# 10XGenomics/rust-pseudoaligner

Measured on AMD Instinct MI355X. Metric: reads/sec pseudoaligned (whole node) on synthetic 150bp reads, higher is better.
Workload: dtype u64; 1 GPU; config3: ~202k-transcript synthetic GENCODE-scale index (K=24), error-free 150bp reads; read_len=150, k=24, transcripts=201914, kmers=103866252, index_bytes=7185579820

## Files before the change

### __graft_entry__.py

```python
from __future__ import annotations

import importlib
import sys
from pathlib import Path

ROOT = Path(__file__).resolve().parent
for p in (str(ROOT), str(ROOT / "tests")):
    if p not in sys.path:
        sys.path.insert(0, p)


def build() -> None:
    _b = importlib.import_module("rust-pseudoaligner_amd._build")
    _b.build_product()
    _b.build_maxbins_variant()
    _b.build_abi_check()
    import helpers
    helpers.build_all()
    pa = helpers.pa
    assert pa.lib().pa_abi_version() == 1


def smoke() -> None:
    import numpy as np
    import helpers
    pa = helpers.pa
    if pa.lib().pa_device_count() < 1:
        raise RuntimeError("smoke() needs a GPU: %s" % pa.lib().pa_last_error().decode())
    host = pa.build_index(str(helpers.FASTA), 20, 8)
    aligner = pa.Pseudoaligner(host, 0)
    ids, seqs = helpers.read_fastq()
    res, coff, cids = aligner.map_batch(seqs)
    o_res, o_coff, o_ids, _ = helpers.Oracle(host).map_reads(seqs, 2, 4)
    helpers.assert_same_as_oracle(res, coff, cids, o_res, o_coff, o_ids, "smoke small.fq K=20")
    r = aligner.map_read("GGCTGTCAACCAGTCCATAGGCAGGGCCATCAGGCACCAAAGGGATTCTGCCAGCATAGT")
    assert r == ([1, 30], 60), r
    print("smoke ok: %d reads bit-exact vs oracle, %d mapped" % (len(seqs), int((res["mismatches"] >> 31).sum())))


if __name__ == "__main__":
    build()
    if "--smoke" in sys.argv:
        smoke()
```

### rust-pseudoaligner_amd/_build.py

```python
from __future__ import annotations

import os
import shutil
import subprocess
from pathlib import Path

PKG = Path(__file__).resolve().parent
ROOT = PKG.parent
CSRC = PKG / "csrc"

PRODUCT_SO = PKG / "libpseudoaligner_amd.so"

HOST_SOURCES = ["host_index.cpp", "dbg_build.cpp", "device_flatten.cpp", "synth.cpp", "fastq_text.cpp", "fastq_reads.cpp", "pair_reader.cpp", "fastq_cells.cpp", "fastq_pairs.cpp", "record_stream.cpp", "host_batch.cpp", "bgzf.cpp", "bus_host.cpp", "bus_correct_host.cpp", "bus_knee_host.cpp", "genes_host.cpp", "window_feed.cpp", "text_window.cpp"]
HIP_SOURCES = ["kernels.hip", "map_pool.hip", "device_index.hip", "map_batch.hip", "device_plumbing.hip", "collective.hip", "barcode_counts.hip", "index_build.hip", "index_fill.hip", "count_sort.hip", "resolve.hip", "render.hip", "fastq_scan.hip", "compact.hip", "quant.hip", "quant_boot.hip", "pairs.hip", "strands.hip", "inflate.hip", "bus.hip", "pair_scan.hip", "genes.hip", "bus_correct.hip", "bus_knee.hip"]


EXTRA_FLAGS = {"map_pool.hip": ["-mllvm", "-disable-machine-sink"]}


def _stale(target: Path, sources) -> bool:
    if not target.exists():
        return True
    t = target.stat().st_mtime
    return any(Path(s).stat().st_mtime > t for s in sources)


def _run(cmd):
    proc = subprocess.run(cmd, capture_output=True, text=True)
    if proc.returncode != 0:
        raise RuntimeError("build failed: %s\n%s\n%s" % (" ".join(map(str, cmd)), proc.stdout, proc.stderr))
    return proc


def hipcc_path() -> str:
    for cand in (shutil.which("hipcc"), "/opt/rocm/bin/hipcc"):
        if cand and os.path.exists(cand):
            return cand
    raise RuntimeError("hipcc not found: the product library cannot be built")


OBJ_DIR = PKG / "_build"


def _deps_of(src: Path):
    return [src] + list(CSRC.glob("*.hpp")) + list(CSRC.glob("*.inc")) + [ROOT / "include" / "pseudoaligner_amd.h", Path(__file__)]


def build_product(force: bool = False) -> Path:
    from concurrent.futures import ThreadPoolExecutor
    srcs = [CSRC / s for s in HOST_SOURCES + HIP_SOURCES]
    OBJ_DIR.mkdir(exist_ok=True)
    hipcc = hipcc_path()
    flags = ["--offload-arch=gfx950", "-O3", "-std=c++17", "-fPIC", "-pthread", "-Wall", "-Wno-unused-function"]
    jobs = []
    for s in srcs:
        obj = OBJ_DIR / (s.name + ".o")
        if force or _stale(obj, _deps_of(s)):
            jobs.append([hipcc] + flags + EXTRA_FLAGS.get(s.name, []) + ["-x", "hip", "-c", str(s), "-o", str(obj)])
    if jobs:
        with ThreadPoolExecutor(max_workers=min(len(jobs), os.cpu_count() or 1)) as ex:
            list(ex.map(_run, jobs))
    objs = [OBJ_DIR / (s.name + ".o") for s in srcs]
    if jobs or _stale(PRODUCT_SO, objs):
        _run([hipcc, "--offload-arch=gfx950", "-shared", "-fPIC", "-pthread"] + [str(o) for o in objs] + ["-ldl", "-lz", "-o", str(PRODUCT_SO)])
    return PRODUCT_SO


MAXBINS_SO = OBJ_DIR / "libpseudoaligner_amd_maxbins2.so"


def build_maxbins_variant(force: bool = False) -> Path:
    build_product()
    hipcc = hipcc_path()
    src = CSRC / "count_sort.hip"
    obj = OBJ_DIR / "count_sort.maxbins2.o"
    if force or _stale(obj, _deps_of(src)):
        _run([hipcc, "--offload-arch=gfx950", "-O3", "-std=c++17", "-fPIC", "-pthread", "-Wall", "-Wno-unused-function", "-DPA_MAX_BINS=2", "-x", "hip", "-c", str(src), "-o", str(obj)])
    objs = [OBJ_DIR / (s + ".o") for s in HOST_SOURCES + HIP_SOURCES if s != "count_sort.hip"] + [obj]
    if force or _stale(MAXBINS_SO, objs):
        _run([hipcc, "--offload-arch=gfx950", "-shared", "-fPIC", "-pthread"] + [str(o) for o in objs] + ["-ldl", "-lz", "-o", str(MAXBINS_SO)])
    return MAXBINS_SO


ABI_CHECK_SRC = ROOT / "integration" / "c" / "abi_check.c"
ABI_CHECK_BIN = ROOT / "integration" / "c" / "abi_check"


def build_abi_check(force: bool = False) -> Path:
    if force or _stale(ABI_CHECK_BIN, [ABI_CHECK_SRC, ROOT / "include" / "pseudoaligner_amd.h", PRODUCT_SO]):
        _run(["gcc", "-std=c11", "-O1", "-Wall", "-Wextra", "-Werror", "-I", str(ROOT / "include"), str(ABI_CHECK_SRC), "-L", str(PKG),
              "-lpseudoaligner_amd", "-Wl,-rpath," + str(PKG), "-Wl,-rpath,$ORIGIN/../../rust-pseudoaligner_amd", "-o", str(ABI_CHECK_BIN)])
    return ABI_CHECK_BIN


if __name__ == "__main__":
    import sys
    if "--list" in sys.argv:
        for s in HOST_SOURCES + HIP_SOURCES:
            print(" ".join([s] + EXTRA_FLAGS.get(s, [])))
    else:
        print(build_product("--force" in sys.argv))
```

### rust-pseudoaligner_amd/csrc/device_flatten.cpp

```cpp
#include "device_flatten.hpp"

#include <algorithm>
#include <atomic>
#include <thread>

#include "dict_slots.hpp"
#include "lane_steps.hpp"
#include "pa_common.hpp"

#ifndef PA_BRANCH_TAILS
#define PA_BRANCH_TAILS 1
#endif

namespace pa {

DevIndexView FlatDevice::host_view() const {
    DevIndexView v;
    v.table = table.data();
    v.nbuckets = nbuckets;
    v.blobs = blobs.data();
    v.ledge = ledge.data();
    v.seg_g = seg_g.data();
    v.seg_nid = seg_nid.data();
    v.ec = ec.data();
    v.class_ref = class_ref.data();
    v.class_len = class_len.data();
    v.wtable = wtable.data();
    v.wbuckets = wbuckets;
    v.kmask = kmer_mask(k);
    v.kmask_hi = k > 32 ? kmer_mask(k - 32) : 0;
    v.k = k;
    v.num_nodes = num_nodes;
    v.num_classes = num_classes;
    v.num_segs = (uint32_t)seg_g.size();
    v.stream_nt = 0;
    v.bitmap_min = bitmap_min;
    v.bitmap_words = bitmap_words;
    return v;
}

namespace {

template <class F>
void par_ranges(int threads, uint64_t n, F f) {
    if (threads <= 1 || n < 4096) { f(0, n, 0); return; }
    std::vector<std::thread> th;
    for (int t = 0; t < threads; ++t) th.emplace_back([=] { f(n * t / threads, n * (t + 1) / threads, t); });
    for (auto& x : th) x.join();
}

template <class KT> struct Dict;

template <>
struct Dict<u128> {
    static constexpr double LOAD = 1.0 / 3.0;
    static constexpr uint32_t SLOTS = 2;
    uint32_t* words;
    uint64_t nbuckets;
    uint64_t bucket_of(u128 kmer) const { return ((pa_mix128((uint64_t)kmer, (uint64_t)(kmer >> 64)) >> 32) * (uint64_t)(uint32_t)nbuckets) >> 32; }
    void insert_mt(u128 kmer, uint32_t handle, uint32_t off) {
        uint64_t b = bucket_of(kmer);
        for (;;) {
            uint32_t* line = words + b * BUCKET_WORDS;
            for (uint32_t i = 0; i < SLOTS; ++i) {
                uint32_t expect = NO_HANDLE;
                if (__atomic_compare_exchange_n(&line[8 * i + 4], &expect, handle, false, __ATOMIC_RELAXED, __ATOMIC_RELAXED)) {
                    line[8 * i] = (uint32_t)kmer; line[8 * i + 1] = (uint32_t)(kmer >> 32);
                    line[8 * i + 2] = (uint32_t)(kmer >> 64); line[8 * i + 3] = (uint32_t)(kmer >> 96);
                    line[8 * i + 5] = off;
                    return;
                }
            }
            if (++b == nbuckets) b = 0;
        }
    }
    void insert_rest_mt(u128, uint32_t, uint32_t) {}
    bool find(u128 kmer, uint32_t& handle, uint32_t& off, uint32_t* probes_out = nullptr) const {
        uint64_t b = bucket_of(kmer);
        for (uint64_t probes = 0; probes < nbuckets; ++probes) {
            const uint32_t* line = words + b * BUCKET_WORDS;
            bool full = true;
            for (uint32_t i = 0; i < SLOTS; ++i) {
                if (line[8 * i + 4] == NO_HANDLE) { full = false; continue; }
                if (line[8 * i] == (uint32_t)kmer && line[8 * i + 1] == (uint32_t)(kmer >> 32) && line[8 * i + 2] == (uint32_t)(kmer >> 64) &&
                    line[8 * i + 3] == (uint32_t)(kmer >> 96)) {
                    handle = line[8 * i + 4];
                    off = line[8 * i + 5];
                    if (probes_out) *probes_out = (uint32_t)probes;
                    return true;
                }
            }
            if (!full) return false;
            if (++b == nbuckets) b = 0;
        }
        return false;
    }
};

struct HostAtomics {
    static bool cas(uint32_t* p, uint32_t expect, uint32_t v) { return __atomic_compare_exchange_n(p, &expect, v, false, __ATOMIC_RELAXED, __ATOMIC_RELAXED); }
    static void and_(uint32_t* p, uint32_t m) { __atomic_fetch_and(p, m, __ATOMIC_RELAXED); }
};

template <>
struct Dict<uint64_t> {
    static constexpr double LOAD = DICT_LOAD;
    static constexpr uint32_t SLOTS = SLOTS_PER_BUCKET;
    uint32_t* words;
    uint64_t nbuckets;
    void insert_mt(uint64_t kmer, uint32_t handle, uint32_t off) { dict_insert_home<HostAtomics>(words, (uint32_t)nbuckets, kmer, handle, off); }
    void insert_rest_mt(uint64_t kmer, uint32_t handle, uint32_t off) { dict_insert_rest<HostAtomics>(words, (uint32_t)nbuckets, kmer, handle, off); }
    bool find(uint64_t kmer, uint32_t& handle, uint32_t& off, uint32_t* probes_out = nullptr) const {
        uint32_t probes = 0;
        const bool found = dict_find64(words, (uint32_t)nbuckets, kmer, handle, off, probes);
        if (probes_out) *probes_out = probes;
        return found;
    }
};

}

template <class KT>
struct KmerMap {
    std::vector<KT> keys;
    std::vector<uint32_t> vals;
    uint64_t mask;
    explicit KmerMap(uint32_t n) {
        uint64_t cap = 16;
        while (cap < 2ull * n + 2) cap <<= 1;
        keys.assign(cap, 0);
        vals.assign(cap, NO_HANDLE);
        mask = cap - 1;
    }
    void insert(KT km, uint32_t v) {
        for (uint64_t j = KmerOps<KT>::hash(km) & mask;; j = (j + 1) & mask) {
            if (vals[j] == NO_HANDLE) { keys[j] = km; vals[j] = v; return; }
            if (keys[j] == km) return;
        }
    }
    uint32_t find(KT km) const {
        for (uint64_t j = KmerOps<KT>::hash(km) & mask;; j = (j + 1) & mask) {
            if (vals[j] == NO_HANDLE) return NO_HANDLE;
            if (keys[j] == km) return vals[j];
        }
    }
};

template <class KT>
static int flatten_t(const pa_flat_index& f, int threads, FlatDevice& out, bool device_dict) {
    if (threads < 1) threads = 1;
    const uint32_t k = f.k, N = f.num_nodes;
    out = FlatDevice();
    out.k = k;
    out.num_nodes = N;
    out.num_classes = f.num_classes;
    const KT mask = KmerOps<KT>::mask(k);
    const uint32_t topshift = 2 * (k - 1);

    if (f.num_transcripts >= 0xFFFFFFFFu) return fail(PA_ERR_UNSUPPORTED, "too many transcripts");
    std::vector<U4> cwin(f.num_classes, U4{0, 0, 0, 0});
    uint64_t nwin = 0;
    for (uint32_t c = 0; c < f.num_classes; ++c) {
        const uint32_t* ids = f.ec_ids + f.ec_offset[c];
        const uint64_t len = f.ec_offset[c + 1] - f.ec_offset[c];
        if (len == 0) continue;
        U4 w{ids[0], 0, 0, 0};
        uint64_t j = 0;
        for (; j < len && ids[j] - w.x < CLASS_WINDOW; ++j) w.y |= 1u << (ids[j] - w.x);
        if (j < len) {
            w.z = ids[j];
            for (; j < len && ids[j] - w.z < CLASS_WINDOW; ++j) w.w |= 1u << (ids[j] - w.z);
        }
        if (j < len) continue;
        cwin[c] = w;
        ++nwin;
    }
    uint32_t id_span = f.num_transcripts;
    for (uint64_t j = 0; j < f.ec_offset[f.num_classes]; ++j) id_span = std::max(id_span, f.ec_ids[j] + 1u);
    out.bitmap_words = ((id_span + 31) / 32 + 2 + 3) & ~3u;
    out.bitmap_min = 16;
    for (;;) {
        uint64_t n = 0;
        for (uint32_t c = 0; c < f.num_classes; ++c)
            n += cwin[c].y == 0 && f.ec_offset[c + 1] - f.ec_offset[c] >= out.bitmap_min;
        out.num_bitmaps = n;
        if (n * out.bitmap_words * 4ull <= (4ull << 30)) break;
        if (out.bitmap_min >= (1u << 24)) { out.bitmap_min = 0; out.num_bitmaps = 0; break; }
        out.bitmap_min *= 2;
    }
    out.class_ref.resize(f.num_classes);
    out.class_len.resize(f.num_classes);
    for (uint32_t c = 0; c < f.num_classes; ++c) {
        const uint64_t len = f.ec_offset[c + 1] - f.ec_offset[c];
        if (len >= 0xFFFFFFFFull || out.ec.size() / 4 >= 0xFFFFFFFFull) return fail(PA_ERR_UNSUPPORTED, "class id lists too large");
        out.class_ref[c] = (uint32_t)(out.ec.size() / 4);
        out.class_len[c] = (uint32_t)len;
        out.max_class_len = std::max(out.max_class_len, (uint32_t)len);
        out.ec.push_back(c);
        out.ec.insert(out.ec.end(), f.ec_ids + f.ec_offset[c], f.ec_ids + f.ec_offset[c + 1]);
        while (out.ec.size() % 4 || out.ec.size() - 4ull * out.class_ref[c] < 8) out.ec.push_back(0xFFFFFFFFu);
        if (out.bitmap_min && cwin[c].y == 0 && len >= out.bitmap_min) {
            const size_t at = out.ec.size();
            if (at != class_bitmap(out.class_ref[c], (uint32_t)len)) return fail(PA_ERR_INTERNAL, "class record of %llu ids is not %u chunks", (unsigned long long)len, class_record_chunks((uint32_t)len));
            out.ec.resize(at + out.bitmap_words, 0u);
            for (uint64_t j = f.ec_offset[c]; j < f.ec_offset[c + 1]; ++j) {
                out.ec[at + (f.ec_ids[j] >> 5)] |= 1u << (f.ec_ids[j] & 31u);
            }
        }
    }
    out.ec.resize(out.ec.size() + 8, 0xFFFFFFFFu);
    out.wbuckets = (uint32_t)std::max<uint64_t>(1, (uint64_t)((double)nwin / (WT_ENTRIES * 0.5)) + 1);
    out.wtable.assign((size_t)out.wbuckets * 16, 0);
    for (uint64_t l = 0; l < out.wbuckets; ++l) out.wtable[l * 16 + 4] = out.wtable[l * 16 + 9] = out.wtable[l * 16 + 14] = NO_CLASS;
    for (uint32_t c = 0; c < f.num_classes; ++c) {
        const U4 w = cwin[c];
        if (w.y == 0) continue;
        uint64_t line = ((uint64_t)window_hash(w.x, w.y, w.z, w.w) * out.wbuckets) >> 32;
        for (bool done = false; !done;) {
            uint32_t* e = out.wtable.data() + line * 16;
            for (uint32_t t = 0; t < WT_ENTRIES && !done; ++t)
                if (e[5 * t + 4] == NO_CLASS) {
                    e[5 * t] = w.x; e[5 * t + 1] = w.y; e[5 * t + 2] = w.z; e[5 * t + 3] = w.w; e[5 * t + 4] = c;
                    done = true;
                }
            if (++line == out.wbuckets) line = 0;
        }
    }

    std::vector<uint64_t> seq_pad(f.node_seq, f.node_seq + (f.seq_bases + 31) / 32);
    seq_pad.resize(seq_pad.size() + 3, 0);
    const uint64_t* node_seq = seq_pad.data();
    uint64_t nk = 0;
    for (uint32_t i = 0; i < N; ++i) {
        if (f.node_len[i] < k) return fail(PA_ERR_FORMAT, "node %u shorter than k", i);
        if (f.node_len[i] >= (1u << 24)) return fail(PA_ERR_UNSUPPORTED, "node %u longer than 2^24 bases", i);
        if (f.node_colour[i] >= f.num_classes) return fail(PA_ERR_FORMAT, "node %u: colour out of range", i);
        nk += f.node_len[i] - k + 1;
    }
    out.num_kmers = nk;
    std::vector<uint32_t> redge(4ull * N, NO_HANDLE), ledge_n(4ull * N, NO_HANDLE);
    {
        KmerMap<KT> first_of(N), last_of(N);
        if (!f.node_redge || !f.node_ledge)
            for (uint32_t i = 0; i < N; ++i) {
                first_of.insert(KmerOps<KT>::get(node_seq, f.node_start[i], k), i);
                last_of.insert(KmerOps<KT>::get(node_seq, f.node_start[i] + f.node_len[i] - k, k), i);
            }
        std::atomic<uint32_t> dangling{NO_HANDLE};
        par_ranges(threads, N, [&](uint64_t a, uint64_t b, int) {
            for (uint64_t i = a; i < b; ++i) {
                const uint64_t s = f.node_start[i];
                const KT first = KmerOps<KT>::get(node_seq, s, k), last = KmerOps<KT>::get(node_seq, s + f.node_len[i] - k, k);
                for (uint32_t base = 0; base < 4; ++base) {
                    if (f.node_exts[i] & (1u << base)) {
                        const uint32_t t = f.node_redge ? f.node_redge[4 * i + base] : first_of.find((last >> 2) | ((KT)base << topshift));
                        if (t >= N) dangling.store((uint32_t)i);
                        else redge[4 * i + base] = t;
                    }
                    if (f.node_exts[i] & (1u << (4 + base))) {
                        const uint32_t t = f.node_ledge ? f.node_ledge[4 * i + base] : last_of.find(((first << 2) | (KT)base) & mask);
                        if (t >= N) dangling.store((uint32_t)i);
                        else ledge_n[4 * i + base] = t;
                    }
                }
            }
        });
        if (dangling.load() != NO_HANDLE)
// ... 108 lines not shown
                        const uint64_t c = 1 + shared_ids(f.node_colour[cur], f.node_colour[t]);
                        if (c > best) { best = c; bn = t; }
                    }
                }
                if (bn == NO_HANDLE) break;
                const uint64_t sb = (uint64_t)fin.back().e - (k - 1), full = sb + f.node_len[bn];
                if ((uint64_t)fin.back().e + 1 >= limit) break;
                const bool cut = full > limit;
                fin.back().branch = branch;
                if (!fits_after(fin, c0, SegI{bn, (uint32_t)sb, (uint32_t)(cut ? limit : full), cut})) { fin.back().branch = false; break; }
                if (cut) break;
                cur = bn;
            }
            for (const size_t c1 = c0 + (chain_first[c + 1] - chain_first[c]); fin.size() > c1 && !fin.back().link;) {
                const uint32_t re = f.node_exts[fin.back().node] & 15u;
                if (re == 0 || (re & (re - 1)) || out.node_s[redge[4 * fin.back().node + (uint32_t)__builtin_ctz(re)]] == 0) break;
                bool done = false;
                if (fin.back().e >= fin[fin.size() - 2].e + 2) {
                    SegI g = fin.back();
                    g.e -= 1;
                    g.link = true;
                    fin.pop_back();
                    done = fits_after(fin, c0, g);
                    if (!done) { g.e += 1; g.link = false; fin.push_back(g); }
                }
                if (!done) { fin.pop_back(); fin.back().branch = false; }
            }
        }
        fin_first.push_back((uint32_t)fin.size());
        segs.swap(fin);
        chain_first.swap(fin_first);
    }
    const size_t nsegs = segs.size();

    std::vector<uint32_t> chain_handle(nchains);
    out.seg_g.resize(nsegs);
    out.seg_nid.resize(nsegs);
    uint64_t cursor = 0;
    for (uint32_t c = 0; c < nchains; ++c) {
        if (cursor >= NO_HANDLE - 8) return fail(PA_ERR_UNSUPPORTED, "graph exceeds the 512 GiB chain address space");
        chain_handle[c] = (uint32_t)cursor;
        for (uint32_t t = chain_first[c]; t < chain_first[c + 1]; ++t) {
            out.seg_g[t] = ((uint64_t)cursor << CH_STRIDE_LOG2) + segs[t].s;
            out.seg_nid[t] = segs[t].node;
        }
        cursor += (segs[chain_first[c + 1] - 1].e + CH_STRIDE - 1) >> CH_STRIDE_LOG2;
    }
    for (uint32_t i = 0; i < N; ++i) out.handle[i] = chain_handle[out.handle[i]];
    const uint64_t nblocks = cursor;
    out.blobs.assign(nblocks * CH_BLOCK + 64, 0);

    std::atomic<uint32_t> bad_edge{NO_HANDLE}, bad_slots{NO_HANDLE};
    par_ranges(threads, nchains, [&](uint64_t ca, uint64_t cb, int) {
        std::vector<uint64_t> cs;
        for (uint64_t c = ca; c < cb; ++c) {
            const uint32_t t0 = chain_first[c], t1 = chain_first[c + 1], clen = segs[t1 - 1].e;
            cs.assign((clen + 31) / 32 + 9, 0);
            for (uint32_t t = t0; t < t1; ++t) {
                const SegI& g = segs[t];
                const uint64_t src = f.node_start[g.node];
                for (uint32_t o = t == t0 ? 0 : k - 1; g.s + o < g.e; ++o) set_base(cs.data(), g.s + o, get_base(node_seq, src + o));
            }
            const uint32_t nblk = (clen + CH_STRIDE - 1) >> CH_STRIDE_LOG2;
            uint32_t tlo = t0;
            for (uint32_t j = 0; j < nblk; ++j) {
                const uint32_t base = j << CH_STRIDE_LOG2;
                uint8_t* blk = out.blobs.data() + ((uint64_t)chain_handle[c] + j) * CH_BLOCK;
                uint32_t* sl = reinterpret_cast<uint32_t*>(blk);
                uint64_t* sq = reinterpret_cast<uint64_t*>(blk + CH_SEQ_BYTES);
                while (tlo < t1 && segs[tlo].e <= base) ++tlo;
                uint32_t slot = 0, recmask = 0;
                for (uint32_t t = tlo; t < t1 && segs[t].s < base + CH_WINDOW; ++t) {
                    const SegI& g = segs[t];
                    const U4 cw = cwin[f.node_colour[g.node]];
                    const bool wide = is_wide(g.node), last = t + 1 == t1, reach = g.e - base < CH_WINDOW,
                               edges = ((last && !g.link && has_redge(g.node)) || g.branch) && reach, link = last && g.link && reach;
                    if (slot + 1 + (wide ? 1 : 0) + (edges || link ? 1 : 0) > CH_SLOTS) { bad_slots.store(g.node); break; }
                    recmask |= 1u << slot;
                    uint32_t* r = sl + 4 * slot++;
                    r[0] = std::min<uint32_t>(g.e - base, SEG_E_FAR) | (wide ? SEG_WIDE : 0u) | (last ? SEG_LAST : 0u) | (edges ? SEG_EDGES : 0u) | (link ? SEG_LINK : 0u);
                    r[1] = f.node_colour[g.node]; r[2] = cw.x; r[3] = cw.y;
                    if (wide) {
                        uint32_t* x = sl + 4 * slot++;
                        x[0] = cw.z; x[1] = cw.w; x[2] = out.class_ref[f.node_colour[g.node]]; x[3] = out.class_len[f.node_colour[g.node]];
                    }
                    if (edges) {
                        uint32_t* x = sl + 4 * slot++;
                        for (uint32_t b = 0; b < 4; ++b) {
                            const uint32_t tn = redge[4 * g.node + b];
                            if (tn != NO_HANDLE && out.node_s[tn] != 0) bad_edge.store(g.node);
                            x[b] = tn == NO_HANDLE ? NO_HANDLE : out.handle[tn];
                        }
                    }
                    if (link) {
                        uint32_t* x = sl + 4 * slot++;
                        const uint32_t xt = out.node_s[g.node] + (g.e - g.s), adv = (xt - 1) >> CH_STRIDE_LOG2;
                        x[0] = out.handle[g.node] + adv;
                        x[1] = xt - (adv << CH_STRIDE_LOG2);
                        x[2] = x[3] = 0;
                    }
                }
                sl[0] |= (std::min(j, CH_BACK_MAX) << SEG_BACK_SHIFT) | (recmask << SEG_RECMASK_SHIFT);
                for (uint32_t w = 0; w < CH_WINDOW / 32; ++w) sq[w] = window32(cs.data(), base + 32ull * w);
            }
        }
    });
    if (bad_slots.load() != NO_HANDLE) return fail(PA_ERR_INTERNAL, "node %u: a chain block needs more than its four slots", bad_slots.load());
    par_ranges(threads, nblocks, [&](uint64_t ba, uint64_t bb, int) {
        for (uint64_t b = ba; b < bb; ++b) {
            uint32_t* sl = reinterpret_cast<uint32_t*>(out.blobs.data() + b * CH_BLOCK);
            const uint32_t recmask = sl[0] >> SEG_RECMASK_SHIFT;
            for (uint32_t t = 0; t < CH_SLOTS; ++t) {
                if (!((recmask >> t) & 1u) || !(sl[4 * t] & SEG_LINK)) continue;
                uint32_t* x = sl + 4 * (t + 1 + ((sl[4 * t] & SEG_WIDE) ? 1u : 0u));
                x[2] = of_cur(block_slot_of(out.blobs.data() + (uint64_t)x[0] * CH_BLOCK, x[1] - 1), true);
            }
        }
    });
    if (bad_edge.load() != NO_HANDLE) return fail(PA_ERR_FORMAT, "node %u: a right edge does not lead to the first k-mer of a chain", bad_edge.load());

    out.ledge.assign(8ull * nblocks + 8, NO_HANDLE);
    for (uint32_t c = 0; c < nchains; ++c) {
        const uint32_t a = segs[chain_first[c]].node;
        for (uint32_t b = 0; b < 4; ++b) {
            const uint32_t tn = ledge_n[4 * a + b];
            uint32_t* e = out.ledge.data() + 8ull * chain_handle[c] + 2 * b;
            e[1] = 0;
            if (tn == NO_HANDLE) continue;
            const uint32_t y = out.node_s[tn] + f.node_len[tn] - k;
            const uint32_t jy = y >> CH_STRIDE_LOG2, j = jy > CH_BACK_MAX ? jy - CH_BACK_MAX : 0;
            e[0] = out.handle[tn] + j;
            e[1] = y - (j << CH_STRIDE_LOG2) + 1;
        }
    }

    auto node_kmers = [&](uint32_t i, auto&& fn) {
        const uint64_t s = f.node_start[i];
        const uint32_t n = f.node_len[i] - k + 1;
        KT km = KmerOps<KT>::get(node_seq, s, k);
        for (uint32_t o = 0; o < n; ++o) {
            if (o) km = (km >> 2) | ((KT)get_base(node_seq, s + o + k - 1) << topshift);
            const uint32_t c = out.node_s[i] + o, blk = out.handle[i] + (c >> CH_STRIDE_LOG2);
            fn(km, blk, dict_entry_off(c, o == 0, block_slot_of(out.blobs.data() + (uint64_t)blk * CH_BLOCK, (c & (CH_STRIDE - 1)) + k - 1)));
        }
    };
    Dict<KT> dict{nullptr, 0};
    if (device_dict) {
        out.node_kcum.resize((size_t)N + 1);
        out.node_kcum[0] = 0;
        for (uint32_t i = 0; i < N; ++i) out.node_kcum[i + 1] = out.node_kcum[i] + (f.node_len[i] - k + 1);
    }
    double load0 = Dict<KT>::LOAD;
    if (const char* v = knob_str("PA_DICT_LOAD")) { const double x = atof(v); if (x > 0.01 && x <= 0.95) load0 = x; }
    for (double load = load0; !device_dict; load *= 0.75) {
        out.nbuckets = std::max<uint64_t>(1, (uint64_t)((double)nk / (Dict<KT>::SLOTS * load)) + 1);
        if (out.nbuckets >= 0xFFFFFFFFull) return fail(PA_ERR_UNSUPPORTED, "dictionary exceeds 2^32 buckets");
        out.table.assign(out.nbuckets * BUCKET_WORDS, 0xFFFFFFFFu);
        dict = Dict<KT>{out.table.data(), out.nbuckets};
        par_ranges(threads, N, [&](uint64_t a, uint64_t b, int) {
            for (uint64_t i = a; i < b; ++i) node_kmers((uint32_t)i, [&](KT km, uint32_t h, uint32_t o) { dict.insert_mt(km, h, o); });
        });
        par_ranges(threads, N, [&](uint64_t a, uint64_t b, int) {
            for (uint64_t i = a; i < b; ++i) node_kmers((uint32_t)i, [&](KT km, uint32_t h, uint32_t o) { dict.insert_rest_mt(km, h, o); });
        });
        std::atomic<uint32_t> bad{NO_HANDLE}, far{0};
        par_ranges(threads, N, [&](uint64_t a, uint64_t b, int) {
            for (uint64_t i = a; i < b; ++i)
                node_kmers((uint32_t)i, [&](KT km, uint32_t h, uint32_t o) {
                    uint32_t fh, fo, probes = 0;
                    if (!dict.find(km, fh, fo, &probes) || fh != h || fo != o) bad.store((uint32_t)i);
                    if (probes > DICT_MAX_PROBES) far.store(1);
                });
        });
        if (bad.load() != NO_HANDLE) return fail(PA_ERR_FORMAT, "a k-mer of node %u occurs twice in the graph", bad.load());
        if (!far.load()) break;
    }
    return PA_OK;
}

int flatten_for_device(const pa_flat_index& f, int threads, FlatDevice& out, bool device_dict) {
    if (f.k < PA_MIN_K || f.k > PA_MAX_K) return fail(PA_ERR_UNSUPPORTED, "k=%u outside [%u,%u]", f.k, PA_MIN_K, PA_MAX_K);
    return f.k <= 32 ? flatten_t<uint64_t>(f, threads, out, device_dict) : flatten_t<u128>(f, threads, out, device_dict);
}

}
```

### rust-pseudoaligner_amd/csrc/device_flatten.hpp

```cpp
#pragma once
#include <vector>

#include "device_layout.hpp"
#ifdef __HIPCC__
#include "hip_buffer.hpp"
#endif

namespace pa {

struct FlatDevice {
    std::vector<uint32_t> table;
    uint64_t nbuckets = 0;
    std::vector<uint8_t> blobs;
    std::vector<uint32_t> handle;
    std::vector<uint32_t> node_s;
    std::vector<uint32_t> ledge;
    std::vector<uint64_t> seg_g;
    std::vector<uint32_t> seg_nid;
    uint32_t num_chains = 0;
    std::vector<uint32_t> ec;
    std::vector<uint32_t> class_ref, class_len;
    std::vector<uint32_t> wtable;
    uint32_t wbuckets = 0;
    uint64_t num_kmers = 0;
    uint32_t k = 0, num_nodes = 0, num_classes = 0, max_class_len = 0;
    uint32_t bitmap_min = 0, bitmap_words = 0;
    uint64_t num_bitmaps = 0;
    std::vector<uint64_t> node_kcum;
    DevIndexView host_view() const;
};

int flatten_for_device(const pa_flat_index& f, int threads, FlatDevice& out, bool device_dict = false);

#ifdef __HIPCC__
int device_fill_index(const FlatDevice& fd, const uint8_t* d_blobs, DeviceBuffer<uint32_t>& table, uint64_t* nbuckets);
#endif

}
```

### rust-pseudoaligner_amd/csrc/device_index.hip

```cpp
#include <hip/hip_runtime.h>

#include <algorithm>
#include <cstdlib>
#include <cstring>
#include <thread>

#include "device_flatten.hpp"
#include "device_index.hpp"
#include "lane_steps.hpp"

using namespace pa;

namespace {

uint64_t list_hash_host(const uint32_t* v, uint32_t n) {
    uint64_t h = 0x243f6a8885a308d3ull ^ n;
    for (uint32_t i = 0; i < n; ++i) h = mix64(h ^ v[i]) + 0x9e3779b97f4a7c15ull;
    return h;
}

}

namespace pa {

void LaunchCtx::release() {
    if (side) (void)hipStreamSynchronize(side);
    ctl.release();
    for (DeviceBuffer<uint32_t>* b : {&spill, &trace, &novel, &keys, &keys_sorted, &keys_ctl, &defer}) b->release();
    for (hipEvent_t e : {ev0, ev1, ev2, ev3, fork, join})
        if (e) (void)hipEventDestroy(e);
    ev0 = ev1 = ev2 = ev3 = fork = join = nullptr;
    if (side) (void)hipStreamDestroy(side);
    side = nullptr;
    timed = false;
}

void* Parked::take(std::mutex& mu) {
    std::lock_guard<std::mutex> g(mu);
    if (held.empty()) return nullptr;
    void* obj = held.back().first;
    held.pop_back();
    return obj;
}
void Parked::put(std::mutex& mu, void* obj, void (*free_fn)(void*)) {
    {
        std::lock_guard<std::mutex> g(mu);
        if (held.size() < cap) {
            held.emplace_back(obj, free_fn);
            return;
        }
    }
    free_fn(obj);
}

void index_host_classes(const pa_index* idx, const uint32_t** ec, const uint32_t** class_ref, int* device) {
    *ec = idx->h_ec.data();
    *class_ref = idx->h_class_ref.data();
    *device = idx->device;
}
void index_pair_view(pa_index* idx, PairIndexView* out) {
    std::lock_guard<std::mutex> g(idx->mu);
    *out = PairIndexView{idx->dv, idx->d_class_table.get(), idx->class_table_size, idx->ovf, idx->device, idx->num_cus};
}
void index_host_class_text(pa_index* idx, const uint64_t** off, const char** text) {
    std::call_once(idx->class_text_once, [idx] {
        const uint32_t nc = idx->stats.num_classes;
        const uint32_t* ec = idx->h_ec.data();
        const uint32_t* cref = idx->h_class_ref.data();
        auto digits = [](uint32_t v) { uint32_t d = 1; while (v >= 10) { v /= 10; ++d; } return d; };
        std::vector<uint64_t>& off_v = idx->h_class_text_off;
        off_v.assign((size_t)nc + 1, 0);
        const int T = std::max(1, std::min(16, usable_threads()));
        const uint32_t* clen = idx->h_class_len.data();
        auto ids_of = [&](uint32_t c, const uint32_t*& ids, uint32_t& n) {
            ids = ec + 4ull * cref[c] + 1;
            n = clen[c];
        };
        {
            std::vector<std::thread> th;
            for (int t = 0; t < T; ++t)
                th.emplace_back([&, t] {
                    for (uint64_t c = (uint64_t)nc * t / T; c < (uint64_t)nc * (t + 1) / T; ++c) {
                        const uint32_t* ids; uint32_t n;
                        ids_of((uint32_t)c, ids, n);
                        uint64_t len = n ? 2ull * (n - 1) : 0;
                        for (uint32_t j = 0; j < n; ++j) len += digits(ids[j]);
                        off_v[c + 1] = len;
                    }
                });
            for (auto& x : th) x.join();
        }
        for (uint32_t c = 0; c < nc; ++c) off_v[c + 1] += off_v[c];
        idx->h_class_text.resize(off_v[nc] + 16);
        {
            std::vector<std::thread> th;
            for (int t = 0; t < T; ++t)
                th.emplace_back([&, t] {
                    for (uint64_t c = (uint64_t)nc * t / T; c < (uint64_t)nc * (t + 1) / T; ++c) {
                        const uint32_t* ids; uint32_t n;
                        ids_of((uint32_t)c, ids, n);
                        char* o = idx->h_class_text.data() + off_v[c];
                        for (uint32_t j = 0; j < n; ++j) {
                            if (j) { *o++ = ','; *o++ = ' '; }
                            char b[10]; int k = 10; uint32_t v = ids[j];
                            do { b[--k] = (char)('0' + v % 10); v /= 10; } while (v);
                            memcpy(o, b + k, (size_t)(10 - k)); o += 10 - k;
                        }
                    }
                });
            for (auto& x : th) x.join();
        }
    });
    *off = idx->h_class_text_off.data();
    *text = idx->h_class_text.data();
}
int index_device_class_text(pa_index* idx, const uint64_t** d_off, const uint8_t** d_text) {
    const uint64_t* off = nullptr;
    const char* txt = nullptr;
    index_host_class_text(idx, &off, &txt);
    std::lock_guard<std::mutex> g(idx->mu);
    if (!idx->d_class_text.get()) {
        if (hipSetDevice(idx->device) != hipSuccess) return fail(PA_ERR_HIP, "hipSetDevice failed");
        int e = upload(idx->d_class_text_off, off, idx->h_class_text_off.size());
        if (e == PA_OK) e = upload(idx->d_class_text, reinterpret_cast<const uint8_t*>(txt), idx->h_class_text.size());
        if (e != PA_OK) return e;
    }
    *d_off = idx->d_class_text_off.get();
    *d_text = idx->d_class_text.get();
    return PA_OK;
}
void* index_take_ingest_cache(pa_index* idx) { return idx->ingest_caches.take(idx->mu); }
void index_put_ingest_cache(pa_index* idx, void* cache, void (*free_fn)(void*)) { idx->ingest_caches.put(idx->mu, cache, free_fn); }
void* index_take_host_pipe(pa_index* idx) { return idx->host_pipes.take(idx->mu); }
void index_put_host_pipe(pa_index* idx, void* pipe, void (*free_fn)(void*)) { idx->host_pipes.put(idx->mu, pipe, free_fn); }

}

extern "C" {

void pa_index_destroy(pa_index* idx) {
    if (!idx) return;
    (void)hipSetDevice(idx->device);
    {
        std::vector<std::pair<void*, void (*)(void*)>> parked;
        { std::lock_guard<std::mutex> g(idx->mu); parked.swap(idx->ingest_caches.held); parked.insert(parked.end(), idx->host_pipes.held.begin(), idx->host_pipes.held.end()); idx->host_pipes.held.clear(); }
        for (auto& c : parked) c.second(c.first);
    }
    for (auto& kv : idx->ctxs) kv.second->release();
    delete idx;
}

int pa_index_create(const pa_flat_index* flat, int device, pa_index** out) {
    if (!flat || !out) return fail(PA_ERR_INVALID_ARG, "null argument");
    int rc = use_device(device);
    if (rc != PA_OK) return rc;
    FlatDevice fd;
    int threads = usable_threads();
    if (threads < 1) threads = 1;
    rc = flatten_for_device(*flat, threads, fd, true);
    if (rc != PA_OK) return rc;

    std::vector<uint32_t> ctab((size_t)fd.num_classes * 2 + 16, 0xFFFFFFFFu);
    for (uint32_t c = 0; c < fd.num_classes; ++c) {
        uint64_t j = list_hash_host(fd.ec.data() + 4ull * fd.class_ref[c] + 1, fd.class_len[c]) % ctab.size();
        while (ctab[j] != 0xFFFFFFFFu)
            if (++j == ctab.size()) j = 0;
        ctab[j] = c;
    }

    pa_index* idx = new (std::nothrow) pa_index();
    if (!idx) return fail(PA_ERR_OOM, "out of memory");
    idx->device = device;
    hipDeviceProp_t prop;
    if (hipGetDeviceProperties(&prop, device) == hipSuccess) idx->num_cus = prop.multiProcessorCount;
    if (idx->num_cus <= 0) idx->num_cus = 256;
    rc = upload(idx->d_blobs, fd.blobs);
    if (rc == PA_OK) rc = upload(idx->d_ledge, fd.ledge);
    if (rc == PA_OK) rc = device_fill_index(fd, idx->d_blobs.get(), idx->d_table, &fd.nbuckets);
    if (rc == PA_OK) rc = upload(idx->d_seg_g, fd.seg_g);
    if (rc == PA_OK) rc = upload(idx->d_seg_nid, fd.seg_nid);
    if (rc == PA_OK) rc = upload(idx->d_ec, fd.ec);
    if (rc == PA_OK) rc = upload(idx->d_class_ref, fd.class_ref);
    if (rc == PA_OK) rc = upload(idx->d_class_len, fd.class_len);
    if (rc == PA_OK) rc = upload(idx->d_class_table, ctab);
    if (rc == PA_OK) rc = upload(idx->d_wtable, fd.wtable);
    if (rc != PA_OK) { pa_index_destroy(idx); return rc; }
    idx->class_table_size = ctab.size();
    idx->dv = fd.host_view();
    idx->dv.table = idx->d_table.get();
    idx->dv.blobs = idx->d_blobs.get();
    idx->dv.ledge = idx->d_ledge.get();
    idx->dv.seg_g = idx->d_seg_g.get();
    idx->dv.seg_nid = idx->d_seg_nid.get();
    idx->h_ec = fd.ec;
    idx->h_class_ref = fd.class_ref;
    idx->h_class_len = fd.class_len;
    idx->dv.ec = idx->d_ec.get();
    idx->dv.class_ref = idx->d_class_ref.get();
    idx->dv.class_len = idx->d_class_len.get();
    idx->dv.wtable = idx->d_wtable.get();
    idx->dv.stream_nt = (fd.k <= 32 && fd.nbuckets * BUCKET_WORDS * 4 > (512ull << 20)) ? 1u : 0u;
    pa_index_stats& s = idx->stats;
    s.num_kmers = fd.num_kmers;
    s.table_slots = fd.nbuckets * SLOTS_PER_BUCKET;
    s.bytes_table = fd.nbuckets * BUCKET_WORDS * 4;
    s.bytes_graph = fd.blobs.size() + fd.ledge.size() * 4 + fd.seg_g.size() * 12;
    s.bytes_classes = (fd.ec.size() + fd.class_ref.size() + fd.class_len.size() + ctab.size() + fd.wtable.size()) * 4;
    s.bytes_total = s.bytes_table + s.bytes_graph + s.bytes_classes;
    s.num_nodes = fd.num_nodes;
    s.num_classes = fd.num_classes;
    s.k = fd.k;
    s.max_class_len = fd.max_class_len;
    *out = idx;
    return PA_OK;
}

int pa_index_create_multi(const pa_flat_index* flat, const int* devices, int ndev, pa_index** out) {
    if (!flat || !devices || !out || ndev < 1) return fail(PA_ERR_INVALID_ARG, "null argument or ndev < 1");
    for (int i = 0; i < ndev; ++i) out[i] = nullptr;
    for (int i = 0; i < ndev; ++i) {
        for (int j = 0; j < i; ++j)
            if (devices[j] == devices[i]) {
                for (int t = 0; t < i; ++t) { pa_index_destroy(out[t]); out[t] = nullptr; }
                return fail(PA_ERR_INVALID_ARG, "device %d listed twice", devices[i]);
            }
        const int rc = pa_index_create(flat, devices[i], &out[i]);
        if (rc != PA_OK) {
            const std::string why = last_error_ref();
            for (int t = 0; t <= i; ++t) { pa_index_destroy(out[t]); out[t] = nullptr; }
            return fail(rc, "device %d: %s", devices[i], why.c_str());
        }
    }
    return PA_OK;
}

int pa_index_get_stats(const pa_index* idx, pa_index_stats* stats) {
    if (!idx || !stats) return fail(PA_ERR_INVALID_ARG, "null argument");
    *stats = idx->stats;
    return PA_OK;
}

uint32_t pa_words_per_read(uint32_t max_read_len) { return (max_read_len + 31) / 32 ? (max_read_len + 31) / 32 : 1; }
size_t pa_tiles_words(uint64_t n_reads, uint32_t words_per_read) { return (size_t)((n_reads + 63) / 64) * words_per_read * 64; }

int pa_encode_reads_device(const pa_index* idx, const uint8_t* d_ascii, const uint64_t* d_offsets, uint64_t n_reads,
                           uint32_t words_per_read, uint64_t* d_tiles, uint32_t* d_lens, void* stream) {
    if (!idx || !d_ascii || !d_offsets || !d_tiles || !d_lens || words_per_read == 0) return fail(PA_ERR_INVALID_ARG, "null argument");
    PA_HIP_TRY(hipSetDevice(idx->device));
    const int e = launch_encode(d_ascii, d_offsets, n_reads, words_per_read, d_tiles, d_lens, static_cast<hipStream_t>(stream));
    if (e) return fail(PA_ERR_HIP, "encode launch: %s", hipGetErrorString((hipError_t)e));
    return PA_OK;
}

}

namespace pa {

static int env_int(const char* name, int dflt) { return knob_int(name, dflt); }

uint32_t spill_cap_of(uint32_t wpr) { return 256 * wpr + 24; }

static int pool_geometry(pa_index* idx, uint64_t n_reads, uint32_t wpr, uint32_t* grid, size_t* lds, uint32_t* slots) {
    const size_t cu_lds = 160 * 1024 - 4096;
    int per_cu = env_int("PA_MAP_BLOCKS_PER_CU", 3);
    uint32_t S = 0;
    for (; per_cu >= 1; --per_cu) {
        const size_t per_wave = cu_lds / (size_t)per_cu / (PA_MAP_BLOCK / 64);
        const size_t per_slot = pool_slot_bytes(wpr);
        if (per_wave < pool_fixed_bytes() + 64 * per_slot + 16) continue;
        S = (uint32_t)((per_wave - pool_fixed_bytes() - 16) / per_slot);
        break;
    }
    if (S < 64) return fail(PA_ERR_UNSUPPORTED, "reads of %u words do not fit the LDS of a compute unit", wpr);
    if (S > pool_max_slots()) S = pool_max_slots();
    const int want = env_int("PA_POOL_SLOTS", 0);
    if (want >= 64 && (uint32_t)want <= S) S = (uint32_t)want;
    *slots = S;
    *lds = pool_lds_bytes(wpr, S);
    int occ = 0;
    if (pool_kernel_occupancy(*lds, &occ) == 0 && occ >= 1 && occ < per_cu) per_cu = occ;
    const uint64_t ntiles = (n_reads + 63) / 64;
    const uint64_t waves_wanted = (ntiles + 7) / 8;
    uint64_t blocks = (waves_wanted + PA_MAP_BLOCK / 64 - 1) / (PA_MAP_BLOCK / 64);
    const uint64_t cap = (uint64_t)idx->num_cus * per_cu;
    if (blocks > cap) blocks = cap;
    if (blocks < 1) blocks = 1;
    *grid = (uint32_t)blocks;
    return PA_OK;
}

static int ctx_of(pa_index* idx, hipStream_t stream, std::shared_ptr<LaunchCtx>* out) {
    std::lock_guard<std::mutex> g(idx->mu);
    auto it = idx->ctxs.find(stream);
    if (it == idx->ctxs.end()) {
        std::shared_ptr<LaunchCtx> c(new (std::nothrow) LaunchCtx());
        if (!c) return fail(PA_ERR_OOM, "out of memory");
        const int rc = grow(c->ctl, 2);
        if (rc != PA_OK) return rc;
        it = idx->ctxs.emplace(stream, std::move(c)).first;
    }
    *out = it->second;
    return PA_OK;
}

int StreamCtx::open(pa_index* idx, hipStream_t stream) {
    PA_HIP_TRY(hipSetDevice(idx->device));
    const int rc = ctx_of(idx, stream, &cx);
    if (rc != PA_OK) return rc;
    lock = std::unique_lock<std::mutex>(cx->mu);
    return PA_OK;
}

int map_launch_locked(pa_index* idx, LaunchCtx* cx, hipStream_t stream, const MapLaunch& m) {
    const uint64_t n_reads = m.n_reads;
    const uint32_t wpr = m.wpr;
    MapCtl* const ctl = cx->ctl.get();
    if (n_reads >= 0xFFFFFFFFull) return fail(PA_ERR_UNSUPPORTED, "at most 2^32-2 reads per batch");
    if (wpr == 0 || wpr > (PA_MAX_READ_LEN + 31) / 32) return fail(PA_ERR_UNSUPPORTED, "words_per_read %u outside [1,%u]", wpr, (PA_MAX_READ_LEN + 31) / 32);
    uint32_t grid = 0;
    size_t lds = 0;
    uint32_t slots = 64;
    int rc = pool_geometry(idx, n_reads, wpr, &grid, &lds, &slots);
    if (rc != PA_OK) return rc;
    const uint32_t spill_cap = spill_cap_of(wpr);
    {
        const size_t per_block = (size_t)(PA_MAP_BLOCK / 64) * slots * spill_cap * 4 * (m.nodes ? 2 : 1);
        const size_t budget = (size_t)6 << 30;
        if ((size_t)grid * per_block > budget) grid = (uint32_t)std::max<size_t>(1, budget / per_block);
    }
    const size_t lanes = (size_t)grid * (PA_MAP_BLOCK / 64) * slots;
    rc = grow(cx->spill, lanes * spill_cap);
    if (rc != PA_OK) return rc;
    if (m.nodes) { rc = grow(cx->trace, lanes * spill_cap); if (rc != PA_OK) return rc; }
    PA_HIP_TRY(hipMemsetAsync(ctl, 0, sizeof(MapCtl), stream));
    MapParams p{};
    p.ix = idx->dv;
    p.tiles = m.tiles;
    p.lens = m.lens;
    p.uniform_len = m.uniform_len;
    p.n_reads = n_reads;
    p.wpr = wpr;
    p.allowed = m.allowed;
    p.results = m.results;
    p.arena = m.arena;
    p.arena_cap = m.arena_cap > PA_MAX_ARENA_ENTRIES ? PA_MAX_ARENA_ENTRIES : m.arena_cap;
    p.colour_out = m.colour;
    p.arena_top = &ctl->arena_top;
    p.status = &ctl->status;
    p.tile_ctr = &ctl->tile_ctr;
    p.spill = cx->spill.get();
    p.spill_cap = spill_cap;
    const uint64_t counts_len = (uint64_t)idx->stats.num_classes + 3;
    const uint64_t defer_cap = defer_capacity(n_reads, grid * (PA_MAP_BLOCK / 64));
    if ((rc = grow(cx->defer, defer_cap * 8))) return rc;
    p.defer = cx->defer.get();
    p.defer_top = &ctl->defer_top;
    p.defer_cap = defer_cap;
    p.keys_cap = 0;
    uint64_t keys_cap = 0;
    if (m.counts) {
        keys_cap = key_stream_capacity(n_reads, grid * (PA_MAP_BLOCK / 64));
        size_t sorted_bytes = 0, ctl_bytes = 0;
        count_keys_scratch(counts_len, n_reads, keys_cap, defer_cap, &sorted_bytes, &ctl_bytes);
        if ((rc = grow(cx->keys, keys_cap + defer_cap)) || (rc = grow(cx->keys_sorted, (sorted_bytes + 3) / 4)) || (rc = grow(cx->keys_ctl, (ctl_bytes + 3) / 4))) return rc;
        p.keys = cx->keys.get();
        p.keys_top = &ctl->keys_top;
        p.keys_cap = keys_cap;
        p.counts = reinterpret_cast<unsigned long long*>(m.counts);
    }
    p.class_table = idx->d_class_table.get();
    p.class_table_size = idx->class_table_size;
    p.pool_slots = slots;
    p.dbg = env_int("PA_MAP_STATS", 0) ? ctl->stats : nullptr;
    p.ablate = (uint32_t)env_int("PA_MAP_ABLATE", 0);
    pa_overflow* ovf = nullptr;
    { std::lock_guard<std::mutex> g(idx->mu); ovf = idx->ovf; }
    if (m.counts && ovf) {
        const uint64_t want = n_reads + 64;
        rc = grow(cx->novel, want * 2);
        if (rc != PA_OK) return rc;
        p.novel_list = cx->novel.get();
        p.novel_ctr = &ctl->novel_ctr;
        p.novel_cap = want;
        overflow_launch_params(ovf, p);
    }
    p.trace = m.nodes ? cx->trace.get() : nullptr;
// ... 215 lines not shown
```

### rust-pseudoaligner_amd/csrc/device_layout.hpp

```cpp
#pragma once
#include <cstdint>

#include "../../include/pseudoaligner_amd.h"

#if defined(__HIPCC__)
#include <hip/hip_runtime.h>
#define PA_HD __host__ __device__ __forceinline__
#else
#define PA_HD inline
#endif

namespace pa {

constexpr uint32_t NO_HANDLE = 0xFFFFFFFFu;
constexpr uint32_t CH_BLOCK = 128;
constexpr uint32_t CH_STRIDE_LOG2 = 6;
constexpr uint32_t CH_STRIDE = 1u << CH_STRIDE_LOG2;
constexpr uint32_t CH_WINDOW = 256;
constexpr uint32_t CH_SLOTS = 4;
constexpr uint32_t CH_SEQ_BYTES = 64;
constexpr uint32_t CH_BACK_MAX = 3;
constexpr uint32_t SEG_E_MASK = 0xFFFFu, SEG_E_FAR = 0xFFFFu;
constexpr uint32_t SEG_WIDE = 1u << 16, SEG_LAST = 1u << 17, SEG_EDGES = 1u << 18, SEG_LINK = 1u << 19;
constexpr uint32_t CH_TAIL = 128;
constexpr uint32_t SEG_BACK_SHIFT = 20, SEG_RECMASK_SHIFT = 28;
constexpr uint32_t ENT_P_MASK = 63u, ENT_NODE_START = 64u, ENT_BACK_SHIFT = 7, ENT_CUR_SHIFT = 9;
PA_HD uint32_t block_slot_of(const uint8_t* blk, uint32_t y) {
    const uint32_t* sl = reinterpret_cast<const uint32_t*>(blk);
    const uint32_t recmask = sl[0] >> SEG_RECMASK_SHIFT;
    for (uint32_t t = 0; t < CH_SLOTS; ++t)
        if (((recmask >> t) & 1u) && (sl[4 * t] & SEG_E_MASK) > y) return t;
    return 0;
}
PA_HD uint32_t dict_entry_off(uint32_t c, bool node_start, uint32_t slot) {
    const uint32_t j = c >> CH_STRIDE_LOG2;
    return (c & ENT_P_MASK) | (node_start ? ENT_NODE_START : 0u) | ((j < CH_BACK_MAX ? j : CH_BACK_MAX) << ENT_BACK_SHIFT) | (slot << ENT_CUR_SHIFT);
}
constexpr uint32_t CLASS_WINDOW = 32;
constexpr uint32_t SLOTS_PER_BUCKET = 4;
constexpr uint32_t BUCKET_WORDS = 16;
constexpr uint32_t SLOT_WORDS = 4;
constexpr uint32_t SLOT_OFF_MASK = 0xFFFFFFu;
constexpr uint32_t SLOT_FLAG_SHIFT = 24;
constexpr uint32_t SLOT_FLAG_OVERFLOW = 8u;
constexpr double DICT_LOAD = 0.25;
constexpr uint32_t DICT_MAX_PROBES = 15;

struct alignas(16) U4 {
    uint32_t x, y, z, w;
};
struct alignas(8) Q2 {
    uint64_t a, b;
};

constexpr uint32_t WT_ENTRIES = 3;

struct DevIndexView {
    const uint32_t* table;
    uint64_t nbuckets;
    const uint8_t* blobs;
    const uint32_t* ledge;
    const uint64_t* seg_g;
    const uint32_t* seg_nid;
    const uint32_t* ec;
    const uint32_t* class_ref;
    const uint32_t* class_len;
    const uint32_t* wtable;
    uint32_t wbuckets;
    uint64_t kmask;
    uint64_t kmask_hi;
    uint32_t k;
    uint32_t num_nodes, num_classes;
    uint32_t num_segs;
    uint32_t stream_nt;
    uint32_t bitmap_min;
    uint32_t bitmap_words;
};

PA_HD uint32_t class_record_chunks(uint32_t len) { return len < 4 ? 2u : (len + 4) >> 2; }
PA_HD uint64_t class_bitmap(uint32_t ref, uint32_t len) { return 4ull * ((uint64_t)ref + class_record_chunks(len)); }

}
```

### rust-pseudoaligner_amd/csrc/dict_slots.hpp

```cpp
#pragma once
#include "lane_steps.hpp"

namespace pa {

template <class A>
PA_HD bool slot_claim(uint32_t* slot, uint64_t km, uint32_t handle, uint32_t off) {
    if (!A::cas(slot + 2, NO_HANDLE, handle)) return false;
    slot[0] = (uint32_t)km;
    slot[1] = (uint32_t)(km >> 32);
    A::and_(slot + 3, off | ~SLOT_OFF_MASK);
    return true;
}

template <class A>
PA_HD void dict_insert_home(uint32_t* table, uint32_t nbuckets, uint64_t km, uint32_t handle, uint32_t off) {
    uint32_t home;
    const uint32_t b = pa_bucket_home(km, nbuckets, home);
    slot_claim<A>(table + (uint64_t)b * BUCKET_WORDS + SLOT_WORDS * home, km, handle, off);
}

template <class A>
PA_HD void dict_insert_rest(uint32_t* table, uint32_t nbuckets, uint64_t km, uint32_t handle, uint32_t off) {
    uint32_t home;
    uint32_t b = pa_bucket_home(km, nbuckets, home);
    {
        const uint32_t* hs = table + (uint64_t)b * BUCKET_WORDS + SLOT_WORDS * home;
        if (hs[2] != NO_HANDLE && hs[0] == (uint32_t)km && hs[1] == (uint32_t)(km >> 32)) return;
    }
    for (bool first = true;; first = false) {
        uint32_t* line = table + (uint64_t)b * BUCKET_WORDS;
        uint32_t* hs = line + SLOT_WORDS * home;
        if (!first && slot_claim<A>(hs, km, handle, off)) return;
        for (uint32_t i = 0; i < 3; ++i)
            if (slot_claim<A>(line + SLOT_WORDS * ((home + 1 + i) & 3u), km, handle, off)) {
                A::and_(hs + 3, ~(1u << (SLOT_FLAG_SHIFT + i)));
                return;
            }
        A::and_(hs + 3, ~(SLOT_FLAG_OVERFLOW << SLOT_FLAG_SHIFT));
        if (++b == nbuckets) b = 0;
    }
}

PA_HD bool dict_find64(const uint32_t* table, uint32_t nbuckets, uint64_t km, uint32_t& handle, uint32_t& off, uint32_t& probes) {
    uint32_t home;
    uint32_t b = pa_bucket_home(km, nbuckets, home);
    const uint32_t klo = (uint32_t)km, khi = (uint32_t)(km >> 32);
    for (probes = 0; probes < nbuckets; ++probes) {
        const uint32_t* line = table + (uint64_t)b * BUCKET_WORDS;
        const U4 v = *reinterpret_cast<const U4*>(line + SLOT_WORDS * home);
        if (slot_holds(v, klo, khi)) { handle = v.z; off = v.w & SLOT_OFF_MASK; return true; }
        const uint32_t fl = slot_flags(v);
        for (uint32_t c = fl & 7u; c; c &= c - 1) {
            const U4 v2 = *reinterpret_cast<const U4*>(line + SLOT_WORDS * ((home + 1 + pa_ctz32(c)) & 3u));
            if (slot_holds(v2, klo, khi)) { handle = v2.z; off = v2.w & SLOT_OFF_MASK; return true; }
        }
        if (!(fl & SLOT_FLAG_OVERFLOW)) return false;
        if (++b == nbuckets) b = 0;
    }
    return false;
}

}
```

### rust-pseudoaligner_amd/csrc/index_fill.hip

```cpp
#include <hip/hip_runtime.h>
#include <cstdlib>

#include <algorithm>

#include "device_flatten.hpp"
#include "dict_slots.hpp"
#include "hip_buffer.hpp"
#include "lane_steps.hpp"
#include "pa_common.hpp"

namespace pa {
namespace {

__device__ __forceinline__ uint64_t win32(const uint64_t* w, uint32_t pos) {
    const uint32_t i = pos >> 5, s = (pos & 31) * 2;
    return s ? (w[i] >> s) | (w[i + 1] << (64 - s)) : w[i];
}

template <class KT> struct FillOps;
template <> struct FillOps<uint64_t> {
    static constexpr uint32_t SLOTS = SLOTS_PER_BUCKET;
    static constexpr double LOAD = DICT_LOAD;
    __host__ __device__ static uint64_t mask(uint32_t k) { return k >= 32 ? ~0ull : ((1ull << (2 * k)) - 1); }
    __device__ static uint64_t get(const uint64_t* seq, uint32_t o, uint32_t k) { return win32(seq, o) & mask(k); }
};
struct DeviceAtomics {
    __device__ static bool cas(uint32_t* p, uint32_t expect, uint32_t v) { return atomicCAS(p, expect, v) == expect; }
    __device__ static void and_(uint32_t* p, uint32_t m) { atomicAnd(p, m); }
};
template <> struct FillOps<u128> {
    static constexpr uint32_t SLOTS = 2;
    static constexpr double LOAD = 1.0 / 3.0;
    __host__ __device__ static u128 mask(uint32_t k) { return k >= 64 ? ~(u128)0 : (((u128)1 << (2 * k)) - 1); }
    __device__ static u128 get(const uint64_t* seq, uint32_t o, uint32_t k) {
        return ((u128)(win32(seq, o + 32) & FillOps<uint64_t>::mask(k - 32)) << 64) | win32(seq, o);
    }
    __device__ static uint32_t bucket(u128 km, uint32_t nbuckets) { return __umulhi((uint32_t)(pa_mix128((uint64_t)km, (uint64_t)(km >> 64)) >> 32), nbuckets); }
    __device__ static bool try_insert(uint32_t* line, u128 km, uint32_t handle, uint32_t off) {
        for (uint32_t i = 0; i < 2; ++i)
            if (atomicCAS(line + 8 * i + 4, NO_HANDLE, handle) == NO_HANDLE) {
                line[8 * i] = (uint32_t)km; line[8 * i + 1] = (uint32_t)(km >> 32);
                line[8 * i + 2] = (uint32_t)(km >> 64); line[8 * i + 3] = (uint32_t)(km >> 96);
                line[8 * i + 5] = off;
                return true;
            }
        return false;
    }
    __device__ static int look(const uint32_t* line, u128 km, uint32_t& handle, uint32_t& off) {
        bool full = true;
        for (uint32_t i = 0; i < 2; ++i) {
            if (line[8 * i + 4] == NO_HANDLE) { full = false; continue; }
            if (line[8 * i] == (uint32_t)km && line[8 * i + 1] == (uint32_t)(km >> 32) && line[8 * i + 2] == (uint32_t)(km >> 64) &&
                line[8 * i + 3] == (uint32_t)(km >> 96)) {
                handle = line[8 * i + 4];
                off = line[8 * i + 5];
                return 1;
            }
        }
        return full ? 2 : 0;
    }
};

template <class KT>
__device__ __forceinline__ bool dict_find(const uint32_t* table, uint32_t nbuckets, KT km, uint32_t& handle, uint32_t& off, uint32_t& probes);
template <>
__device__ __forceinline__ bool dict_find<uint64_t>(const uint32_t* table, uint32_t nbuckets, uint64_t km, uint32_t& handle, uint32_t& off, uint32_t& probes) {
    return dict_find64(table, nbuckets, km, handle, off, probes);
}
template <>
__device__ __forceinline__ bool dict_find<u128>(const uint32_t* table, uint32_t nbuckets, u128 km, uint32_t& handle, uint32_t& off, uint32_t& probes) {
    uint32_t b = FillOps<u128>::bucket(km, nbuckets);
    for (probes = 0; probes < nbuckets; ++probes) {
        const int r = FillOps<u128>::look(table + (uint64_t)b * BUCKET_WORDS, km, handle, off);
        if (r != 2) return r == 1;
        if (++b == nbuckets) b = 0;
    }
    return false;
}

struct KmerAt {
    uint32_t node, block, off;
    const uint64_t* seq;
    uint32_t rel;
};

__device__ __forceinline__ uint32_t node_of_kmer(const uint64_t* kcum, uint32_t num_nodes, uint64_t g) {
    uint32_t lo = 0, hi = num_nodes - 1;
    while (lo < hi) {
        const uint32_t mid = lo + (hi - lo + 1) / 2;
        if (kcum[mid] <= g) lo = mid; else hi = mid - 1;
    }
    return lo;
}

__device__ __forceinline__ KmerAt kmer_at(const uint8_t* blobs, const uint32_t* handle, const uint32_t* node_s, const uint64_t* kcum, uint32_t num_nodes, uint64_t g, uint32_t k) {
    KmerAt a;
    a.node = node_of_kmer(kcum, num_nodes, g);
    const uint32_t o = (uint32_t)(g - kcum[a.node]), c = node_s[a.node] + o;
    a.block = handle[a.node] + (c >> CH_STRIDE_LOG2);
    a.off = dict_entry_off(c, o == 0, block_slot_of(blobs + (uint64_t)a.block * CH_BLOCK, (c & (CH_STRIDE - 1)) + k - 1));
    a.seq = reinterpret_cast<const uint64_t*>(blobs + (uint64_t)a.block * CH_BLOCK + CH_SEQ_BYTES);
    a.rel = c & (CH_STRIDE - 1);
    return a;
}

template <class KT>
__global__ __launch_bounds__(256) void pa_fill_insert_kernel(const uint8_t* __restrict__ blobs, const uint32_t* __restrict__ handle, const uint32_t* __restrict__ node_s,
                                                             const uint64_t* __restrict__ kcum, uint32_t num_nodes, uint64_t nk, uint32_t k, uint32_t* table,
                                                             uint32_t nbuckets, int pass) {
    const uint64_t g = (uint64_t)blockIdx.x * blockDim.x + threadIdx.x;
    if (g >= nk) return;
    const KmerAt a = kmer_at(blobs, handle, node_s, kcum, num_nodes, g, k);
    const KT km = FillOps<KT>::get(a.seq, a.rel, k);
    if constexpr (sizeof(KT) == 8) {
        if (pass == 0) dict_insert_home<DeviceAtomics>(table, nbuckets, km, a.block, a.off);
        else dict_insert_rest<DeviceAtomics>(table, nbuckets, km, a.block, a.off);
    } else {
        if (pass != 0) return;
        uint32_t b = FillOps<KT>::bucket(km, nbuckets);
        for (;;) {
            if (FillOps<KT>::try_insert(table + (uint64_t)b * BUCKET_WORDS, km, a.block, a.off)) return;
            if (++b == nbuckets) b = 0;
        }
    }
}

template <class KT>
__global__ __launch_bounds__(256) void pa_fill_verify_kernel(const uint8_t* __restrict__ blobs, const uint32_t* __restrict__ handle, const uint32_t* __restrict__ node_s,
                                                             const uint64_t* __restrict__ kcum, uint32_t num_nodes, uint64_t nk, uint32_t k,
                                                             const uint32_t* __restrict__ table, uint32_t nbuckets, uint32_t* __restrict__ flags) {
    const uint64_t g = (uint64_t)blockIdx.x * blockDim.x + threadIdx.x;
    if (g >= nk) return;
    const KmerAt a = kmer_at(blobs, handle, node_s, kcum, num_nodes, g, k);
    const KT km = FillOps<KT>::get(a.seq, a.rel, k);
    uint32_t fh = 0, fo = 0, probes = 0;
    if (!dict_find<KT>(table, nbuckets, km, fh, fo, probes) || fh != a.block || fo != a.off) atomicMin(flags, a.node);
    if (probes > DICT_MAX_PROBES) flags[1] = 1;
}

template <class KT>
int fill_t(const FlatDevice& fd, const uint8_t* d_blobs, DeviceBuffer<uint32_t>& table_out, uint64_t* nbuckets_out) {
    const uint32_t N = fd.num_nodes, k = fd.k;
    const uint64_t nk = fd.num_kmers;
    DeviceBuffer<uint32_t> table, d_handle, d_node_s, d_flags;
    DeviceBuffer<uint64_t> d_kcum;
    int e = d_handle.alloc(N ? N : 1);
    if (e == PA_OK) e = d_node_s.alloc(N ? N : 1);
    if (e == PA_OK) e = d_kcum.alloc((size_t)N + 1);
    if (e == PA_OK) e = d_flags.alloc(4);
    if (e != PA_OK) return e;
    if (N) PA_HIP_TRY(hipMemcpy(d_handle.get(), fd.handle.data(), (size_t)N * 4, hipMemcpyHostToDevice));
    if (N) PA_HIP_TRY(hipMemcpy(d_node_s.get(), fd.node_s.data(), (size_t)N * 4, hipMemcpyHostToDevice));
    PA_HIP_TRY(hipMemcpy(d_kcum.get(), fd.node_kcum.data(), ((size_t)N + 1) * 8, hipMemcpyHostToDevice));
    uint64_t nbuckets = 0;
    double load0 = FillOps<KT>::LOAD;
    {
        size_t free_b = 0, total_b = 0;
        const double dense = sizeof(KT) == 8 ? 0.5 : FillOps<KT>::LOAD;
        if (load0 < dense && hipMemGetInfo(&free_b, &total_b) == hipSuccess && (double)nk / (FillOps<KT>::SLOTS * load0) * BUCKET_WORDS * 4 > (double)free_b / 4) load0 = dense;
    }
    if (const char* v = knob_str("PA_DICT_LOAD")) { const double x = atof(v); if (x > 0.01 && x <= 0.95) load0 = x; }
    for (double load = load0;; load *= 0.75) {
        nbuckets = std::max<uint64_t>(1, (uint64_t)((double)nk / (FillOps<KT>::SLOTS * load)) + 1);
        if (nbuckets >= 0xFFFFFFFFull) return fail(PA_ERR_UNSUPPORTED, "dictionary exceeds 2^32 buckets");
        if ((e = table.alloc(nbuckets * BUCKET_WORDS)) != PA_OK) return e;
        PA_HIP_TRY(hipMemsetAsync(table.get(), 0xFF, nbuckets * BUCKET_WORDS * 4, nullptr));
        const uint32_t init[4] = {NO_HANDLE, 0u, NO_HANDLE, NO_HANDLE};
        PA_HIP_TRY(hipMemcpy(d_flags.get(), init, 16, hipMemcpyHostToDevice));
        if (nk) {
            const dim3 grid((uint32_t)((nk + 255) / 256));
            for (int pass = 0; pass < (sizeof(KT) == 8 ? 2 : 1); ++pass) {
                hipLaunchKernelGGL(pa_fill_insert_kernel<KT>, grid, dim3(256), 0, nullptr, d_blobs, d_handle.get(), d_node_s.get(), d_kcum.get(), N, nk, k,
                                   table.get(), (uint32_t)nbuckets, pass);
                PA_HIP_TRY(hipGetLastError());
            }
            hipLaunchKernelGGL(pa_fill_verify_kernel<KT>, grid, dim3(256), 0, nullptr, d_blobs, d_handle.get(), d_node_s.get(), d_kcum.get(), N, nk, k,
                               table.get(), (uint32_t)nbuckets, d_flags.get());
            PA_HIP_TRY(hipGetLastError());
        }
        uint32_t flags[4];
        PA_HIP_TRY(hipMemcpy(flags, d_flags.get(), 16, hipMemcpyDeviceToHost));
        if (flags[0] != NO_HANDLE) return fail(PA_ERR_FORMAT, "a k-mer of node %u occurs twice in the graph", flags[0]);
        if (!flags[1]) break;
    }
    *nbuckets_out = nbuckets;
    table_out = std::move(table);
    return PA_OK;
}

}

int device_fill_index(const FlatDevice& fd, const uint8_t* d_blobs, DeviceBuffer<uint32_t>& table, uint64_t* nbuckets) {
    return fd.k <= 32 ? fill_t<uint64_t>(fd, d_blobs, table, nbuckets) : fill_t<u128>(fd, d_blobs, table, nbuckets);
}

}
```

### rust-pseudoaligner_amd/csrc/lane_steps_body.hpp

```cpp
#if PA_LS_COMMON
enum : uint32_t { ST_EMPTY = 0, ST_SEEK = 1, ST_FWD = 2, ST_LEFT = 3, ST_ISECT = 4, ST_NONE = 5,
                  ST_F_LIGHT = 6, ST_F_SCAN = 7, ST_F_COOP = 8, ST_F_BITS = 9, ST_F_MASK = 10, ST_COUNT = 11 };
enum : uint32_t { F_FRESH = 1u, F_FIRST_SEEK = 2u, F_LEFT_SEED = 4u, F_SPILL_OVERFLOW = 8u, F_CAREFUL = 16u, F_LISTS = 32u,
                  F_SMALL_BASE = 64u,
                  F_SPEC = 128u };
constexpr uint32_t NO_CLASS = 0xFFFFFFFFu;
constexpr uint32_t LDS_CLASSES = 4;
#endif

#if PA_LS_LANE
#if !PA_LANE_WIDE
struct Lane {
    uint32_t rid;
    uint32_t lk;
    uint32_t cm;
    uint32_t h;
    uint32_t of;
    uint32_t rr;
    uint32_t rm;
    uint32_t ph;
    uint32_t nc;
};
constexpr uint32_t LANE_MAX_READ_LEN = 16383u;
PA_HD uint32_t l_L(const Lane& s) { return s.lk & 0x3FFFu; }
// ... 364 lines not shown
        c.wcand[0] = ec_len;
        if (ec_len <= 8) l_or_flags(s, F_SMALL_BASE);
    }
    *reinterpret_cast<U4*>(c.win) = r;
    if (n < LDS_CLASSES) {
        c.refs[n] = ec_ref;
        c.lens[n] = ec_len;
        c.cids[n] = hd.cid;
    } else {
        const uint32_t o = 4 * (n - LDS_CLASSES);
        if (o + 3 >= c.spill_cap || n >= NC_COL_MASK) { l_or_flags(s, F_SPILL_OVERFLOW); return false; }
        c.spill[o] = ec_ref;
        c.spill[o + 1] = ec_len;
        c.spill[o + 2] = hd.cid;
    }
    s.nc += 1;
    return false;
}

PA_HD void lane_start(Lane& s, uint32_t rid, uint32_t L, uint32_t k) {
    s.rid = rid;
    l_zero(s);
    l_set_lk(s, L, 0, L < k ? ST_NONE : ST_SEEK);
    s.of = F_FIRST_SEEK << 24;
}
PA_HD void restart_lists(Lane& s, uint32_t k) {
    lane_start(s, s.rid, l_L(s), k);
    l_or_flags(s, F_LISTS);
}
PA_HD uint32_t window_todo(const Lane& s) {
    const uint32_t n = l_ncol(s);
    return (n >> 1) == 0 ? 0u : (n & 1u) ? 1u : 2u;
}
#endif
#if PA_LS_COMMON
PA_HD void list_window_mask(const DevIndexView& ix, uint32_t ref, uint32_t len, uint32_t b1, uint32_t b2, uint32_t& m1, uint32_t& m2) {
    const uint32_t* ids = ix.ec + 4ull * ref + 1;
    m1 = m2 = 0;
    for (uint32_t j = 0; j < len; ++j) {
        const uint32_t d1 = ids[j] - b1, d2 = ids[j] - b2;
        if (d1 < CLASS_WINDOW) m1 |= 1u << d1;
        if (d2 < CLASS_WINDOW) m2 |= 1u << d2;
    }
#if !defined(__HIP_DEVICE_COMPILE__)
    if (ix.bitmap_min && len >= ix.bitmap_min) {
        const uint32_t* bits = ix.ec + class_bitmap(ref, len);
        const uint32_t x1 = window_bits(bits, b1), x2 = window_bits(bits, b2);
        if (x1 != m1 || x2 != m2) { m1 = m2 = 0xDEADBEEFu; }
    }
#endif
}
#endif
#if PA_LS_LANE
PA_HD void mask_pending(Lane& s, const DevIndexView& ix, ColRef c) {
    U4 w = *reinterpret_cast<const U4*>(c.win);
    const uint32_t np = l_npend(s);
    uint32_t a1 = w.y, a2 = w.w;
    for (uint32_t i = 0; i < np; ++i) {
        uint32_t m1, m2;
        list_window_mask(ix, c.pend[2 * i], c.pend[2 * i + 1], w.x, w.z, m1, m2);
        a1 &= m1;
        a2 &= m2;
    }
    if (a1 != w.y || a2 != w.w) c.wcand[0] = NO_CLASS;
    w.y = a1;
    w.w = a2;
    *reinterpret_cast<U4*>(c.win) = w;
    s.nc = (s.nc & ~NC_COL_MASK) | 1u;
}
#endif

#if PA_LS_COMMON
struct SeekProbe {
    U4 v;
    uint32_t klo, khi;
    uint32_t pending;
};
struct SeekProbe2 {
    U4 k0, v0, k1, v1;
    uint32_t w0, w1, w2, w3;
};
constexpr uint32_t SK_NAMED = 7u, SK_FULL = 8u, SK_MASK = 15u;
PA_HD uint32_t pa_bucket_home(uint64_t kmer, uint32_t nbuckets, uint32_t& home) {
    uint32_t x = (uint32_t)kmer * 0x9E3779B1u + (uint32_t)(kmer >> 32) * 0x85EBCA77u;
    x ^= x >> 15;
    x *= 0x2C1B3C6Du;
    x ^= x >> 13;
    home = x & 3u;
#if defined(__HIP_DEVICE_COMPILE__)
    return __umulhi(x, nbuckets);
#else
    return (uint32_t)(((uint64_t)x * nbuckets) >> 32);
#endif
}
#endif
#if PA_LS_LANE
PA_HD bool seek_two(const Lane& s, uint32_t K) { return (l_flags(s) & F_SPEC) && l_probe(s) == 0 && l_kp(s) + PA_SEEK_STRIDE <= l_L(s) - K; }
PA_HD uint32_t l_pending(const Lane& s) { return s.rm & SK_MASK; }
PA_HD void seek_issue(const Lane& s, const DevIndexView& ix, ReadRef rd, SeekProbe& q, uint32_t ahead = 0, bool live = true) {
    const uint32_t at = live ? l_kp(s) + ahead : l_kp(s);
    const uint64_t kmer = read_window_in(rd, at) & ix.kmask;
    uint32_t home;
    uint32_t b = pa_bucket_home(kmer, (uint32_t)ix.nbuckets, home) + (ahead ? 0u : l_probe(s));
    if (b >= (uint32_t)ix.nbuckets) b -= (uint32_t)ix.nbuckets;
    q.pending = ahead ? 0u : l_pending(s);
    const uint32_t named = q.pending & SK_NAMED;
    uint32_t slot = named ? (home + 1u + pa_ctz32(named)) & 3u : home;
    if (!live) { b = 0; slot = 0; }
    q.v = ld_stream(reinterpret_cast<const U4*>(ix.table + (uint64_t)b * BUCKET_WORDS + SLOT_WORDS * slot), (PA_NT & 4) || ix.stream_nt);
    q.klo = (uint32_t)kmer;
    q.khi = (uint32_t)(kmer >> 32);
}
#endif
#if PA_LS_COMMON
PA_HD bool slot_holds(const U4& v, uint32_t klo, uint32_t khi) { return v.z != NO_HANDLE && v.x == klo && v.y == khi; }
PA_HD uint32_t slot_flags(const U4& v) { return (~v.w >> SLOT_FLAG_SHIFT) & 15u; }
#endif
#if PA_LS_LANE
PA_HD void seek_finish(Lane& s, uint32_t K, uint32_t h, uint32_t off, bool full, uint32_t probe);
#endif
#if PA_LS_COMMON
PA_HD void seek_eval(const SeekProbe& q, uint32_t& h, uint32_t& off, bool& full, uint32_t& pending) {
    h = NO_HANDLE;
    off = 0;
    const bool hit = slot_holds(q.v, q.klo, q.khi);
    if (hit) { h = q.v.z; off = q.v.w & SLOT_OFF_MASK; }
    const uint32_t named = q.pending & SK_NAMED;
    const uint32_t next = named ? (named & (named - 1u)) | (q.pending & SK_FULL) : slot_flags(q.v);
    pending = hit ? 0u : (next & SK_NAMED) ? next : 0u;
    full = (next & SK_FULL) != 0;
}
#endif
#if PA_LS_LANE
PA_HD bool seek_settle(Lane& s, uint32_t K, const SeekProbe& q, bool more) {
    uint32_t h, off, pending;
    bool full;
    seek_eval(q, h, off, full, pending);
    if (pending) { s.rm = (s.rm & ~SK_MASK) | pending; return true; }
    const uint32_t probe = l_probe(s);
    if (!more || h != NO_HANDLE || (full && probe < DICT_MAX_PROBES)) {
        seek_finish(s, K, h, off, full, probe);
        return true;
    }
    l_set_kp(s, l_kp(s) + PA_SEEK_STRIDE);
    s.rm &= ~SK_MASK;
    s.nc &= ~(15u << NC_PROBE_SHIFT);
    return false;
}
PA_HD void seek_complete(Lane& s, uint32_t K, const SeekProbe& q) { (void)seek_settle(s, K, q, false); }
PA_HD void seek_complete2(Lane& s, uint32_t K, const SeekProbe& q0, bool two, const SeekProbe& q1) {
    if (seek_settle(s, K, q0, two)) return;
    (void)seek_settle(s, K, q1, false);
}
PA_HD void seek_finish(Lane& s, uint32_t K, uint32_t h, uint32_t off, bool full, uint32_t probe) {
    const uint32_t L = l_L(s), kp = l_kp(s);
    s.nc &= ~(15u << NC_PROBE_SHIFT);
    s.rm &= ~SK_MASK;
    if (h != NO_HANDLE) {
        s.h = h;
        const uint32_t fl = l_flags(s), p = (off & ENT_P_MASK) | of_cur((off >> ENT_CUR_SHIFT) & 3u, true);
        const uint32_t thr = L / 5;
        if ((fl & F_FIRST_SEEK) && kp >= thr) {
            const uint32_t back = (off >> ENT_BACK_SHIFT) & CH_BACK_MAX;
            l_set_left_ra(s, kp);
            s.ph = h - back;
            s.rr = (off & ENT_P_MASK) + CH_STRIDE * back + ((off & ENT_NODE_START) ? 1u : 0u);
            s.of = p | (((fl & ~(F_FIRST_SEEK | F_SPEC)) | F_FRESH | F_LEFT_SEED) << 24);
            l_set_st(s, ST_LEFT);
        } else {
            s.of = p | (((fl & ~(F_FIRST_SEEK | F_SPEC)) | F_FRESH) << 24);
            l_set_st(s, ST_FWD);
        }
        return;
    }
    if (full && probe < DICT_MAX_PROBES) {
        s.nc |= (probe + 1) << NC_PROBE_SHIFT;
        return;
    }
    const uint32_t nkp = kp + PA_SEEK_STRIDE;
    l_set_kp(s, nkp);
    l_or_flags(s, F_SPEC);
    if (nkp > L - K) l_set_st(s, l_ncol(s) ? ST_ISECT : ST_NONE);
}
#endif

#if PA_LS_COMMON
PA_HD uint64_t pa_mix128(uint64_t lo, uint64_t hi) { return pa_mix64(lo ^ (pa_mix64(hi) * 0x9e3779b97f4a7c15ull)); }
#endif

#if PA_LS_LANE
PA_HD void seek_issue_k2(const Lane& s, const DevIndexView& ix, ReadRef rd, SeekProbe2& q) {
    const uint32_t kp = l_kp(s), probe = l_probe(s);
    const uint64_t klo = read_window(rd, kp), khi = read_window(rd, kp + 32) & ix.kmask_hi;
#if defined(__HIP_DEVICE_COMPILE__)
    uint32_t b = __umulhi((uint32_t)(pa_mix128(klo, khi) >> 32), (uint32_t)ix.nbuckets) + probe;
#else
    uint32_t b = (uint32_t)(((pa_mix128(klo, khi) >> 32) * (uint32_t)ix.nbuckets) >> 32) + probe;
#endif
    if (b >= (uint32_t)ix.nbuckets) b -= (uint32_t)ix.nbuckets;
    const U4* line = reinterpret_cast<const U4*>(ix.table + (uint64_t)b * BUCKET_WORDS);
    q.k0 = line[0]; q.v0 = line[1]; q.k1 = line[2]; q.v1 = line[3];
    q.w0 = (uint32_t)klo; q.w1 = (uint32_t)(klo >> 32); q.w2 = (uint32_t)khi; q.w3 = (uint32_t)(khi >> 32);
}
PA_HD void seek_complete_k2(Lane& s, uint32_t K, const SeekProbe2& q) {
    const bool h0 = q.k0.x == q.w0 && q.k0.y == q.w1 && q.k0.z == q.w2 && q.k0.w == q.w3 && q.v0.x != NO_HANDLE,
               h1 = q.k1.x == q.w0 && q.k1.y == q.w1 && q.k1.z == q.w2 && q.k1.w == q.w3 && q.v1.x != NO_HANDLE;
    seek_finish(s, K, h0 ? q.v0.x : h1 ? q.v1.x : NO_HANDLE, h0 ? q.v0.y : q.v1.y, q.v0.x != NO_HANDLE && q.v1.x != NO_HANDLE, l_probe(s));
}
PA_HD void seek_step(Lane& s, const DevIndexView& ix, ReadRef rd) {
    const uint32_t K = ix.k;
    if (K > 32) {
        SeekProbe2 q2;
        seek_issue_k2(s, ix, rd, q2);
        seek_complete_k2(s, K, q2);
        return;
    }
    SeekProbe q, q1;
    const bool two = seek_two(s, K);
    seek_issue(s, ix, rd, q);
    seek_issue(s, ix, rd, q1, PA_SEEK_STRIDE, two);
    seek_complete2(s, K, q, two, q1);
}
#endif

#if PA_LS_COMMON
struct FwdLoad {
    U4 s0, s1, s2, s3;
    Q2 s01, s23, s45;
};
constexpr uint32_t CH_SEQ_LAST = CH_WINDOW / 32 - 1;
PA_HD const Q2* fwd_seq_pair(const uint64_t* sq, uint32_t w) { return reinterpret_cast<const Q2*>(sq + (w == CH_SEQ_LAST ? CH_SEQ_LAST - 1 : w)); }
PA_HD uint64_t fwd_seq_first(const Q2& v, uint32_t w) { return w == CH_SEQ_LAST ? v.b : v.a; }
PA_HD bool fwd_next_block(uint32_t& h, uint32_t& x, uint32_t rest) {
    const uint32_t adv = x + rest <= CH_WINDOW ? 0u : (x - 1) >> CH_STRIDE_LOG2;
    h += adv;
    x -= adv << CH_STRIDE_LOG2;
    return adv == 0;
}
#endif
#if PA_LS_LANE
PA_HD void fwd_issue(const Lane& s, const DevIndexView& ix, FwdLoad& f) {
    const uint32_t K = ix.k, L = l_L(s);
    const bool fresh = l_flags(s) & F_FRESH;
    const uint32_t xs = l_off(s) + (fresh ? K : 0u);
    const uint32_t kp0 = l_kp(s) + (fresh ? K : 0u);
    const uint8_t* blk = chain_block(ix, s.h);
    const U4* sp = reinterpret_cast<const U4*>(blk);
    const uint32_t rot = l_cur(s);
    f.s0 = PA_LD(8, sp + rot); f.s1 = PA_LD(8, sp + ((rot + 1) & 3u)); f.s2 = PA_LD(8, sp + ((rot + 2) & 3u)); f.s3 = PA_LD(8, sp + ((rot + 3) & 3u));
    const uint32_t most = pa_min(L - kp0, 128u), nwords = ((xs & 31) + most + 31) >> 5, w0 = xs >> 5;
    const uint64_t* sq = reinterpret_cast<const uint64_t*>(blk + CH_SEQ_BYTES);
    f.s01 = PA_LD(8, fwd_seq_pair(sq, w0));
    f.s23 = f.s45 = Q2{0ull, 0ull};
    if (nwords > 2) f.s23 = PA_LD(8, fwd_seq_pair(sq, w0 + 2));
    if (nwords > 4) f.s45.a = PA_LD(8, sq + (w0 + 4));
}
#endif

#if PA_LS_COMMON
struct DiffMasks {
    uint64_t m0, m1, m2, m3;
    uint32_t p0, p1, p2, p3;
};
PA_HD uint64_t diff_word(const DiffMasks& d, uint32_t w) { return sel4q(w, d.m0, d.m1, d.m2, d.m3); }
PA_HD uint32_t mism_prefix(const DiffMasks& d, uint32_t z) {
    const uint32_t w = z >> 5, r = z & 31u;
    const uint32_t b03 = sel4(w, 0u, d.p0, d.p1, d.p2), base = (w & 4u) ? d.p3 : b03;
    return base + pa_popc64(diff_word(d, w) & ((1ull << (2 * r)) - 1));
}
#endif

#if PA_LS_LANE
template <bool TRACE = false>
PA_HD void fwd_finish_general(Lane& s, const DevIndexView& ix, ReadRef rd, ColRef cols, uint32_t allowed, const FwdLoad& f) {
    const uint32_t K = ix.k, L = l_L(s);
    const uint32_t fl = l_flags(s);
    const bool fresh = fl & F_FRESH, careful = fl & F_CAREFUL;
    uint32_t x = l_off(s) + (fresh ? K : 0u);
    uint32_t kp = l_kp(s) + (fresh ? K : 0u);
    const uint32_t xs = x, kp0 = kp;
    uint32_t snp = s.rr >> 24, cov = l_cov(s), mism = l_mism(s);
    const uint32_t most = pa_min(L - kp0, 128u), nwords = ((xs & 31) + most + 31) >> 5;
    const uint64_t a[5] = {fwd_seq_first(f.s01, xs >> 5), f.s01.b, nwords > 2 ? fwd_seq_first(f.s23, (xs >> 5) + 2) : 0ull, nwords > 2 ? f.s23.b : 0ull,
                           nwords > 4 ? f.s45.a : 0ull};
    const Slots sl{f.s0, f.s1, f.s2, f.s3};
    const bool known = s.of & OF_CUR_KNOWN;
    const uint32_t rot = l_cur(s);
    uint32_t cur = known ? 0u : seg_find(sl, x - 1);
    Seg g = seg_at(sl, cur);
    if (fresh) {
        cov += K;
        if (push_node<TRACE>(s, cols, ix, g, 64ull * s.h + l_off(s))) {
            restart_lists(s, K);
            return;
        }
        snp = 0;
    }
    uint64_t r[5];
    {
        const uint32_t i0 = (kp0 >> 5) * rd.stride, ilast = (rd.wmax - 1) * rd.stride;
#pragma unroll
        for (uint32_t i = 0; i < 5; ++i) r[i] = rd.p[pa_min(i0 + i * rd.stride, ilast)];
    }
    const uint32_t sh_a = (xs & 31) * 2, sh_r = (kp0 & 31) * 2;
    DiffMasks dm;
    dm.m0 = diff_mask(funnel(r[0], r[1], sh_r) ^ funnel(a[0], a[1], sh_a), 32u);
    dm.m1 = most > 32u ? diff_mask(funnel(r[1], r[2], sh_r) ^ funnel(a[1], a[2], sh_a), 32u) : 0ull;
    dm.m2 = most > 64u ? diff_mask(funnel(r[2], r[3], sh_r) ^ funnel(a[2], a[3], sh_a), 32u) : 0ull;
    dm.m3 = most > 96u ? diff_mask(funnel(r[3], r[4], sh_r) ^ funnel(a[3], a[4], sh_a), 32u) : 0ull;
    dm.p0 = pa_popc64(dm.m0); dm.p1 = dm.p0 + pa_popc64(dm.m1); dm.p2 = dm.p1 + pa_popc64(dm.m2); dm.p3 = dm.p2 + pa_popc64(dm.m3);
    const uint32_t lim = careful ? 32u : 128u;
    uint32_t consumed = 0, st = ST_FWD, h = s.h, nfl = fl & ~F_FRESH;
    uint32_t ncur = 0xFFFFFFFFu;
    bool premature = false, hopped = false;
    for (;;) {
        const uint32_t n = pa_min(pa_min(g.e - x, L - kp), lim - consumed);
        uint32_t matched;
        if (!careful) {
            const uint32_t cnt = mism_prefix(dm, consumed + n) - mism_prefix(dm, consumed);
            if (snp + cnt > allowed) { nfl |= F_CAREFUL; break; }
            snp += cnt;
            mism += cnt;
            matched = n;
        } else {
            matched = compare_chunk(n ? dm.m0 & (~0ull >> (64u - 2u * n)) : 0ull, n, allowed, snp, mism, premature);
        }
        x += matched; kp += matched; cov += matched; consumed += matched;
        if (premature) { nfl &= ~F_CAREFUL; st = kp > L - K ? ST_ISECT : ST_SEEK; break; }
        if (kp >= L) { nfl &= ~F_CAREFUL; st = ST_ISECT; break; }
        if (x < g.e) break;
        if (g.flags & SEG_LINK) {
            const U4 lk = slot_at(sl, cur + 1 + ((g.flags & SEG_WIDE) ? 1u : 0u));
            h = lk.x;
            x = lk.y;
            ncur = lk.z;
            hopped = true;
            break;
        }
        nfl &= ~F_CAREFUL;
        if (g.flags & SEG_LAST) {
            uint32_t nh = NO_HANDLE;
            if (g.flags & SEG_EDGES) {
                const U4 ed = slot_at(sl, cur + 1 + ((g.flags & SEG_WIDE) ? 1u : 0u));
                const uint32_t b = read_base(rd, kp);
                nh = sel4(b, ed.x, ed.y, ed.z, ed.w);
            }
            if (nh != NO_HANDLE) {
                h = nh;
                x = 0;
                kp -= K - 1;
                cov -= K - 1;
                nfl |= F_FRESH;
                ncur = of_cur(0u, true);
                hopped = true;
            } else st = kp > L - K ? ST_ISECT : ST_SEEK;
            break;
        }
        if (consumed >= 128u) break;
        const bool branch = (g.flags & SEG_EDGES) != 0;
        {
            if ((diff_word(dm, consumed >> 5) >> (2 * (consumed & 31u))) & 1ull) {
                uint32_t nh = NO_HANDLE;
                if (branch) {
                    const U4 ed = slot_at(sl, cur + 1 + ((g.flags & SEG_WIDE) ? 1u : 0u));
                    nh = sel4(read_base(rd, kp), ed.x, ed.y, ed.z, ed.w);
                }
                if (nh != NO_HANDLE) {
                    h = nh;
                    x = 0;
                    kp -= K - 1;
                    cov -= K - 1;
                    nfl |= F_FRESH;
                    ncur = of_cur(0u, true);
                    hopped = true;
// ... 552 lines not shown
```

### rust-pseudoaligner_amd/csrc/map_pool.hip

```cpp
#include <hip/hip_runtime.h>

#include "kernels.hpp"
#include "lane_steps.hpp"
#include "kernel_utils.hpp"

#ifndef PA_FILL
#define PA_FILL 1
#endif
#ifndef PA_COOP_MIN
#define PA_COOP_MIN 2u
#endif
#ifndef PA_REFILL_ALIGN
#define PA_REFILL_ALIGN 1u
#endif
#ifndef PA_RARE_MIN
#define PA_RARE_MIN 16u
#endif

#ifdef PA_ISA_MARKS
#define PA_MARK(name) asm volatile("; PA_MARK " name ::: "memory")
#else
#define PA_MARK(name)
#endif

namespace pa {
namespace {

typedef __attribute__((address_space(3))) uint64_t* lds_u64;
typedef __attribute__((address_space(3))) uint32_t* lds_u32;
typedef __attribute__((address_space(3))) uint8_t* lds_u8;
typedef __attribute__((address_space(3))) uint16_t* lds_u16;
typedef __attribute__((address_space(3))) unsigned long long* lds_u64w;
typedef uint32_t u32x4 __attribute__((ext_vector_type(4)));
typedef __attribute__((address_space(3))) u32x4* lds_v4;
typedef __attribute__((address_space(1))) u32x4* glb_v4w;
typedef __attribute__((address_space(1))) const u32x4* glb_v4;
typedef __attribute__((address_space(1))) uint32_t* glb_u32w;
typedef __attribute__((address_space(1))) const uint32_t* glb_u32;
typedef __attribute__((address_space(1))) unsigned long long* glb_u64w;
__device__ __forceinline__ void store_result(glb_v4w dst, u32x4 v) {
    if (PA_NT & 2) __builtin_nontemporal_store(v, dst);
    else *dst = v;
}

typedef __attribute__((address_space(4))) const MapParams* karg_ptr;

__device__ __forceinline__ DevIndexView view_of(karg_ptr p) {
    DevIndexView v;
    v.table = p->ix.table; v.nbuckets = p->ix.nbuckets; v.blobs = p->ix.blobs; v.ledge = p->ix.ledge;
    v.seg_g = p->ix.seg_g; v.seg_nid = p->ix.seg_nid; v.ec = p->ix.ec; v.class_ref = p->ix.class_ref; v.class_len = p->ix.class_len;
    v.wtable = p->ix.wtable; v.wbuckets = p->ix.wbuckets; v.kmask = p->ix.kmask; v.kmask_hi = p->ix.kmask_hi; v.k = p->ix.k; v.num_nodes = p->ix.num_nodes; v.num_classes = p->ix.num_classes; v.num_segs = p->ix.num_segs; v.stream_nt = p->ix.stream_nt; v.bitmap_min = p->ix.bitmap_min; v.bitmap_words = p->ix.bitmap_words;
    return v;
}

static_assert(ST_NSTAT == ST_COUNT + 4, "kernels.hpp");
constexpr uint32_t ST_DUAL = ST_COUNT;
constexpr uint32_t POOL_FIXED = 960;
constexpr uint32_t POOL_MAX_SLOTS = 128;
constexpr uint32_t LIST_ROW_HDR = 12;

__device__ __forceinline__ uint32_t rank_in(uint64_t m) { return __builtin_amdgcn_mbcnt_hi((uint32_t)(m >> 32), __builtin_amdgcn_mbcnt_lo((uint32_t)m, 0u)); }

__device__ __forceinline__ uint64_t shfl64(uint64_t v, uint32_t src) {
    return ((uint64_t)(uint32_t)__shfl((int)(v >> 32), (int)src, 64) << 32) | (uint32_t)__shfl((int)v, (int)src, 64);
}

__device__ __forceinline__ uint64_t arena_alloc(uint32_t cnt_alloc, uint32_t lane, karg_ptr p, lds_u64w chunk) {
    const uint32_t incl = wave_incl_scan(cnt_alloc);
    const uint32_t total = (uint32_t)__builtin_amdgcn_readlane((int)incl, 63);
    asm volatile("" ::: "memory");
    unsigned long long chunk_cur = chunk[0];
    if (total > 0) {
        if (chunk_cur + total > chunk[1]) {
            const unsigned long long want = total > PA_ARENA_CHUNK ? total : PA_ARENA_CHUNK;
            unsigned long long base = 0;
            if (lane == 0) base = atomicAdd(p->arena_top, want);
            base = ((unsigned long long)(uint32_t)__builtin_amdgcn_readfirstlane((int)(base >> 32)) << 32) | (uint32_t)__builtin_amdgcn_readfirstlane((int)base);
            chunk_cur = base;
            if (lane == 0) chunk[1] = base + want;
        }
        if (lane == 0) chunk[0] = chunk_cur + total;
    }
    asm volatile("" ::: "memory");
    return chunk_cur + (incl - cnt_alloc);
}

constexpr uint32_t NO_KEY = 0xFFFFFFFFu;
__device__ __forceinline__ void append_keys(uint32_t key, uint32_t lane, karg_ptr p, lds_u32 kchunk) {
    const uint64_t m = __ballot(key != NO_KEY);
    if (m == 0) return;
    const uint32_t cnt = (uint32_t)__popcll(m);
    const glb_u32w keys = (glb_u32w)p->keys;
    asm volatile("" ::: "memory");
    const uint32_t cur = kchunk[0], room = kchunk[1] - cur;
    uint32_t nbase = 0;
    if (cnt > room) {
        if (lane == 0) {
            nbase = (uint32_t)atomicAdd(p->keys_top, (unsigned long long)PA_KEY_CHUNK);
            if ((uint64_t)nbase + PA_KEY_CHUNK > p->keys_cap) { atomicOr(p->status, PA_STATUS_SPILL_OVERFLOW); nbase = 0; }
        }
        nbase = (uint32_t)__builtin_amdgcn_readfirstlane((int)nbase);
    }
    const uint32_t r = rank_in(m);
    if (key != NO_KEY) keys[r < room ? cur + r : nbase + (r - room)] = key;
    if (lane == 0) {
        if (cnt > room) { kchunk[0] = nbase + (cnt - room); kchunk[1] = nbase + PA_KEY_CHUNK; }
        else kchunk[0] = cur + cnt;
    }
    asm volatile("" ::: "memory");
}

__device__ __forceinline__ void append_deferred(bool has, u32x4 e0, u32x4 e1, uint32_t lane, karg_ptr p, lds_u32 dchunk) {
    const uint64_t m = __ballot(has);
    if (m == 0) return;
    const uint32_t cnt = (uint32_t)__popcll(m);
    const glb_v4w out = (glb_v4w)p->defer;
    asm volatile("" ::: "memory");
    const uint32_t cur = dchunk[0], room = dchunk[1] - cur;
    uint32_t nbase = 0;
    if (cnt > room) {
        if (lane == 0) {
            nbase = (uint32_t)atomicAdd(p->defer_top, (unsigned long long)PA_DEFER_CHUNK);
            if ((uint64_t)nbase + PA_DEFER_CHUNK > p->defer_cap) { atomicOr(p->status, PA_STATUS_SPILL_OVERFLOW); nbase = 0; }
        }
        nbase = (uint32_t)__builtin_amdgcn_readfirstlane((int)nbase);
    }
    if (has) {
        const uint32_t r = rank_in(m);
        const uint64_t at = 2ull * (r < room ? cur + r : nbase + (r - room));
        out[at] = e0;
        out[at + 1] = e1;
    }
    if (lane == 0) {
        if (cnt > room) { dchunk[0] = nbase + (cnt - room); dchunk[1] = nbase + PA_DEFER_CHUNK; }
        else dchunk[0] = cur + cnt;
    }
    asm volatile("" ::: "memory");
}

__device__ __forceinline__ uint32_t list_hits(glb_u32 ec, uint32_t xref, uint32_t nch, uint32_t maxch, const uint32_t (&b)[8]) {
    const glb_v4 xrec = (glb_v4)(ec + 4ull * xref);
    uint32_t acc = 0;
    for (uint32_t c0 = 0; c0 < maxch; c0 += 4) {
        u32x4 w[4];
#pragma unroll
        for (uint32_t t = 0; t < 4; ++t) w[t] = xrec[c0 + t < nch ? c0 + t : 0];
#pragma unroll
        for (uint32_t t = 0; t < 4; ++t)
            if (c0 + t < nch) {
                const U4 ww{w[t].x, w[t].y, w[t].z, w[t].w};
                acc |= scan_words(ww, c0 + t == 0, b);
            }
    }
    return acc;
}

__device__ __forceinline__ uint32_t wave_max(uint32_t v) {
    for (uint32_t o = 32; o; o >>= 1) v = max(v, (uint32_t)__shfl_xor((int)v, (int)o, 64));
    return (uint32_t)__builtin_amdgcn_readfirstlane((int)v);
}

__device__ __forceinline__ void window_hits(glb_u32 ec, uint32_t xref, uint32_t len, bool act, uint32_t b1, uint32_t b2, uint32_t bitmap_min, uint32_t& m1, uint32_t& m2) {
    const bool bm = act && bitmap_min != 0 && len >= bitmap_min;
    uint32_t bw[4] = {0u, 0u, 0u, 0u};
    if (__ballot(bm)) {
        if (bm) {
            const glb_u32 bits = ec + class_bitmap(xref, len);
            bw[0] = bits[b1 >> 5]; bw[1] = bits[(b1 >> 5) + 1]; bw[2] = bits[b2 >> 5]; bw[3] = bits[(b2 >> 5) + 1];
        }
    }
    act = act && !bm;
    const glb_v4 rec = (glb_v4)(ec + 4ull * xref);
    const uint32_t nch = act ? (len + 4) >> 2 : 0u;
    uint32_t c[2] = {0u, 0u}, e[2] = {nch, 0u};
    const bool lng = act && len > 64;
    if (__ballot(lng)) {
        if (lng) {
            const glb_u32 ids = ec + 4ull * xref + 1;
#pragma unroll
            for (uint32_t r = 0; r < 2; ++r) {
                const uint32_t b = r ? b2 : b1;
                uint32_t lo = 0, hi = len;
                while (lo < hi) {
                    const uint32_t mid = (lo + hi) >> 1;
                    if (ids[mid] < b) lo = mid + 1; else hi = mid;
                }
                c[r] = (1 + lo) >> 2;
                e[r] = min(nch, ((1 + lo + CLASS_WINDOW - 1) >> 2) + 1);
            }
        }
    }
    m1 = m2 = 0;
#pragma unroll
    for (uint32_t r = 0; r < 2; ++r) {
        const uint32_t mx = wave_max(e[r] > c[r] ? e[r] - c[r] : 0u);
        for (uint32_t c0 = 0; c0 < mx; c0 += 4) {
            u32x4 w[4];
#pragma unroll
            for (uint32_t t = 0; t < 4; ++t) w[t] = rec[c[r] + c0 + t < e[r] ? c[r] + c0 + t : 0u];
#pragma unroll
            for (uint32_t t = 0; t < 4; ++t)
                if (c[r] + c0 + t < e[r]) {
                    const uint32_t v[4] = {w[t].x, w[t].y, w[t].z, w[t].w};
#pragma unroll
                    for (uint32_t i = 0; i < 4; ++i) {
                        if (i == 0 && c[r] + c0 + t == 0) continue;
                        const uint32_t d1 = v[i] - b1, d2 = v[i] - b2;
                        if (d1 < CLASS_WINDOW) m1 |= 1u << d1;
                        if (d2 < CLASS_WINDOW) m2 |= 1u << d2;
                    }
                }
        }
    }
    if (bm) {
        m1 = (uint32_t)((((uint64_t)bw[1] << 32) | bw[0]) >> (b1 & 31u));
        m2 = (uint32_t)((((uint64_t)bw[3] << 32) | bw[2]) >> (b2 & 31u));
    }
}

}

namespace narrow {
#define PA_K_WIDE 0
#include "map_pool_kernel.inc"
#undef PA_K_WIDE
}

namespace wide {
#define PA_K_WIDE 1
#include "map_pool_kernel.inc"
#undef PA_K_WIDE
}

size_t pool_slot_bytes(uint32_t wpr) {
    return wpr > PA_LDS_READ_WORDS ? (size_t)wide::SLOT_FIXED_BYTES : 8 * (size_t)wpr + narrow::SLOT_FIXED_BYTES;
}
size_t pool_fixed_bytes() { return POOL_FIXED; }
uint32_t pool_max_slots() { return POOL_MAX_SLOTS; }

size_t pool_lds_bytes(uint32_t wpr, uint32_t slots) {
    const size_t wave_bytes = (POOL_FIXED + (size_t)slots * pool_slot_bytes(wpr) + 15) & ~(size_t)15;
    return wave_bytes * (PA_MAP_BLOCK / 64);
}

template <class K>
static int launch_kernel(K kernel, const MapParams& p, uint32_t grid, size_t lds_bytes, hipStream_t stream) {
    if (lds_bytes > 48 * 1024) {
        const hipError_t e = hipFuncSetAttribute(reinterpret_cast<const void*>(kernel), hipFuncAttributeMaxDynamicSharedMemorySize, (int)lds_bytes);
        if (e != hipSuccess) return (int)e;
    }
    hipLaunchKernelGGL(kernel, dim3(grid), dim3(PA_MAP_BLOCK), lds_bytes, stream, p);
    return (int)hipGetLastError();
}

int launch_map_pool(const MapParams& p, uint32_t grid, size_t lds_bytes, hipStream_t stream) {
    const bool gread = p.wpr > PA_LDS_READ_WORDS;
    if (gread) return p.trace ? launch_kernel(&wide::pa_map_pool_kernel<true, true, false, false>, p, grid, lds_bytes, stream)
                              : launch_kernel(&wide::pa_map_pool_kernel<false, true, false, false>, p, grid, lds_bytes, stream);
    if (p.trace) return launch_kernel(&narrow::pa_map_pool_kernel<true, false, false, false>, p, grid, lds_bytes, stream);
#ifdef PA_DEBUG_KNOBS
    if (p.dbg || p.ablate) return launch_kernel(&narrow::pa_map_pool_kernel<false, false, true, false>, p, grid, lds_bytes, stream);
#endif
    if (p.ix.k > 32)
        return p.pool_slots == 128 ? launch_kernel(&narrow::pa_map_pool_kernel<false, false, false, true, true>, p, grid, lds_bytes, stream)
                                   : launch_kernel(&narrow::pa_map_pool_kernel<false, false, false, false, true>, p, grid, lds_bytes, stream);
    if (p.pool_slots == 128) return launch_kernel(&narrow::pa_map_pool_kernel<false, false, false, true>, p, grid, lds_bytes, stream);
    return launch_kernel(&narrow::pa_map_pool_kernel<false, false, false, false>, p, grid, lds_bytes, stream);
}

int pool_kernel_occupancy(size_t lds_bytes, int* blocks_per_cu) {
    return (int)hipOccupancyMaxActiveBlocksPerMultiprocessor(blocks_per_cu, reinterpret_cast<const void*>(&narrow::pa_map_pool_kernel<false, false, false, false>),
                                                             PA_MAP_BLOCK, lds_bytes);
}

}
```

### rust-pseudoaligner_amd/csrc/map_pool_kernel.inc

```
namespace {

template <bool TRACE>
__device__ __forceinline__ void trace_out(const Lane& s, bool mapped, uint32_t gslot, karg_ptr p) {
    if (!TRACE) return;
    const uint32_t spill_cap = p->spill_cap;
    const uint32_t nt = l_ntrace(s);
    const uint32_t nn = mapped ? (nt < spill_cap ? nt : spill_cap) : 0;
    ((glb_u32w)p->nodes_len)[s.rid] = mapped ? nt : 0;
    const glb_u32w tr = (glb_u32w)p->trace + (uint64_t)gslot * spill_cap;
    const glb_u32w out = (glb_u32w)p->nodes_out + (uint64_t)s.rid * spill_cap;
    for (uint32_t j = 0; j < nn; ++j) out[j] = tr[j];
}

template <bool TRACE>
__device__ __forceinline__ uint32_t emit_record(Lane& s, uint32_t cnt, uint32_t cnt_alloc, uint64_t my_off, uint32_t base_len,
                                                uint32_t base_colour, uint32_t gslot, karg_ptr p, bool& defer) {
    uint32_t colour = NO_CLASS, class_off = (uint32_t)my_off;
    bool novel = false;
    if (my_off + cnt_alloc > p->arena_cap) atomicOr(p->status, PA_STATUS_ARENA_FULL);
    if (cnt == base_len) {
        colour = base_colour;
        class_off = PA_CLASS_REF | base_colour;
    } else novel = cnt != 0;
    if (l_flags(s) & F_SPILL_OVERFLOW) atomicOr(p->status, PA_STATUS_SPILL_OVERFLOW);
    ((glb_v4w)p->results)[s.rid] = u32x4{l_cov(s), l_mism(s) | PA_MAPPED_BIT, class_off, cnt};
    trace_out<TRACE>(s, true, gslot, p);
    const glb_u32w colour_out = (glb_u32w)p->colour_out;
    if (novel && (p->keys != nullptr || colour_out != nullptr) && my_off + cnt_alloc <= p->arena_cap) {
        defer = true;
        s.lk = 0;
        return NO_KEY;
    }
    if (colour_out) colour_out[s.rid] = colour;
    s.lk = 0;
    const uint32_t num_classes = p->ix.num_classes;
    return cnt == 0 ? num_classes + 1 : colour == NO_CLASS ? num_classes : colour;
}

__device__ __forceinline__ uint32_t queue_of(Lane& s, uint32_t K) {
    uint32_t st = l_st(s);
    if (st == ST_ISECT) {
        const uint32_t fl = l_flags(s);
        if (!(fl & F_LISTS)) {
            const uint32_t todo = window_todo(s);
            if (todo == 2) { restart_lists(s, K); return ST_SEEK; }
            st = todo ? ST_F_MASK : ST_F_BITS;
        } else st = l_ncol(s) <= 3 ? ST_F_LIGHT : (fl & F_SMALL_BASE) ? ST_F_SCAN : ST_F_COOP;
        l_set_st(s, st);
    }
    return st == ST_NONE ? (uint32_t)ST_F_BITS : st;
}

template <bool GREAD>
__device__ __forceinline__ void refill_slot(Lane& s, uint64_t rid, uint32_t slot, karg_ptr p, lds_u64 rd, lds_u32 wc, uint32_t S, uint32_t wpr,
                                            uint32_t K) {
    const uint32_t* lens = p->lens;
    uint32_t L = lens ? lens[rid] : p->uniform_len;
    if (L > wpr * 32) L = wpr * 32;
    if (!GREAD) {
        const uint64_t* src = p->tiles + ((rid >> 6) * wpr) * 64 + (rid & 63);
        if (wpr == 5) {
            const bool nt = (PA_NT & 1) || p->ix.stream_nt;
            const uint64_t v0 = ld_stream(src, nt), v1 = ld_stream(src + 64, nt), v2 = ld_stream(src + 128, nt), v3 = ld_stream(src + 192, nt), v4 = ld_stream(src + 256, nt);
            rd[slot] = v0; rd[S + slot] = v1; rd[2 * S + slot] = v2; rd[3 * S + slot] = v3; rd[4 * S + slot] = v4;
        } else if (wpr == 4) {
            const bool nt = (PA_NT & 1) || p->ix.stream_nt;
            const uint64_t v0 = ld_stream(src, nt), v1 = ld_stream(src + 64, nt), v2 = ld_stream(src + 128, nt), v3 = ld_stream(src + 192, nt);
            rd[slot] = v0; rd[S + slot] = v1; rd[2 * S + slot] = v2; rd[3 * S + slot] = v3;
        } else
        for (uint32_t w0 = 0; w0 < wpr; w0 += 8) {
            uint64_t v[8];
#pragma unroll
            for (uint32_t i = 0; i < 8; ++i) v[i] = w0 + i < wpr ? PA_LD(1, src + (uint64_t)(w0 + i) * 64) : 0ull;
#pragma unroll
            for (uint32_t i = 0; i < 8; ++i)
                if (w0 + i < wpr) rd[(w0 + i) * S + slot] = v[i];
        }
    }
    lane_start(s, (uint32_t)rid, L, K);
    wc[2 * slot + 1] = (uint32_t)rid;
}

__device__ __forceinline__ void lane_load(Lane& s, lds_v4 stA, lds_v4 stB, lds_v4 stC, uint32_t slot) {
    const u32x4 a = stA[slot], b = stB[slot];
    s.lk = a.x; s.cm = a.y; s.h = a.z; s.of = a.w; s.rr = b.x; s.rm = b.y; s.ph = b.z; s.nc = b.w;
#if PA_K_WIDE
    const u32x4 c = stC[slot];
    s.xl = c.x; s.xm = c.y; s.xt = c.z;
#else
    (void)stC;
#endif
}
__device__ __forceinline__ void lane_store(const Lane& s, lds_v4 stA, lds_v4 stB, lds_v4 stC, uint32_t slot) {
    stA[slot] = u32x4{s.lk, s.cm, s.h, s.of};
    stB[slot] = u32x4{s.rr, s.rm, s.ph, s.nc};
#if PA_K_WIDE
    stC[slot] = u32x4{s.xl, s.xm, s.xt, 0u};
#else
    (void)stC;
#endif
}
constexpr uint32_t SLOT_FIXED_BYTES = 32 + 16 + 8 + (PA_K_WIDE ? 16 : 0);

}

#ifndef PA_MAP_MIN_BLOCKS
#define PA_MAP_MIN_BLOCKS 3
#endif
template <bool TRACE, bool GREAD, bool DBG, bool S128 = false, bool KBIG = false>
__global__ __launch_bounds__(PA_MAP_BLOCK, PA_MAP_MIN_BLOCKS) void pa_map_pool_kernel(const MapParams p_arg) {
    karg_ptr kp = (karg_ptr)__builtin_amdgcn_kernarg_segment_ptr();
    (void)p_arg;
#define p (*kp)
#define PA_DBG (DBG && p.dbg)
#define PA_ABLATE(bit) (DBG && (p.ablate & (bit)))
    extern __shared__ __attribute__((aligned(16))) uint8_t smem[];
    const uint32_t lane = lane_id();
    const uint32_t wave_in_block = (uint32_t)__builtin_amdgcn_readfirstlane((int)(threadIdx.x >> 6));
    const uint32_t waves_per_block = PA_MAP_BLOCK / 64;
    const uint32_t wave = blockIdx.x * waves_per_block + wave_in_block;
    const uint32_t nwaves = gridDim.x * waves_per_block;
    const uint32_t S = S128 ? 128u : p.pool_slots, wpr = p.wpr;
    const uint32_t lwpr = GREAD ? 0u : wpr;

    const uint32_t wave_bytes = (POOL_FIXED + S * (8 * lwpr + SLOT_FIXED_BYTES) + 15) & ~15u;
    uint8_t* const wbase = smem + wave_in_block * wave_bytes;
    const lds_u64w chunk = (lds_u64w)wbase;
    const lds_u32 dbg = (lds_u32)(wbase + 16);
    const lds_u64w dbg_clk = (lds_u64w)(wbase + 16 + 8 * ST_NSTAT);
    const lds_u32 kchunk = (lds_u32)(wbase + 256);
    const lds_u32 dchunk = (lds_u32)(wbase + 264);
    const lds_u64 rd = (lds_u64)(wbase + POOL_FIXED);
    const lds_v4 stA = (lds_v4)(wbase + POOL_FIXED + 8 * lwpr * S);
    const lds_v4 stB = (lds_v4)(wbase + POOL_FIXED + (8 * lwpr + 16) * S);
    constexpr uint32_t XW = PA_K_WIDE ? 16u : 0u;
    const lds_v4 stC = (lds_v4)(wbase + POOL_FIXED + (8 * lwpr + 32) * S);
    const lds_v4 win = (lds_v4)(wbase + POOL_FIXED + (8 * lwpr + 32 + XW) * S);
    const lds_u32 wc = (lds_u32)(wbase + POOL_FIXED + (8 * lwpr + 48 + XW) * S);
    const lds_u8 sb = (lds_u8)(wbase + 768);
    const lds_u8 poplist = (lds_u8)(wbase + 896);
    if (lane < 64) ((lds_u32)wbase)[lane] = 0;
    if (lane < 4) kchunk[lane] = 0;
    ((lds_u16)sb)[lane] = (uint16_t)((lane < S ? (uint32_t)ST_EMPTY : 0xFFu) | ((lane + 64 < S ? (uint32_t)ST_EMPTY : 0xFFu) << 8));

    const uint32_t ntiles = (uint32_t)((p.n_reads + 63) >> 6);
    const uint32_t chunk_tiles = ntiles / (nwaves * 4) >= 16 ? 16u : ntiles / (nwaves * 4) >= 1 ? ntiles / (nwaves * 4) : 1u;
    uint64_t next = (uint64_t)wave * chunk_tiles << 6;
    uint64_t end = (uint64_t)(wave + 1) * chunk_tiles << 6;
    if (end > p.n_reads) end = p.n_reads;
    if (next > end) next = end;
    bool more = true;
    uint32_t seen = nwaves * chunk_tiles;

    const bool counting = p.keys != nullptr;

#define PA_CNT(t) ((uint32_t)__popcll(__ballot(st_lo == (t))) + (uint32_t)__popcll(__ballot(st_hi == (t))))
#define PA_POP(t, nn, out)                                                                         \
    {                                                                                              \
        const uint64_t m0_ = __ballot(st_lo == (t)), m1_ = __ballot(st_hi == (t));                 \
        const uint32_t r1_ = (uint32_t)__popcll(m0_) + rank_in(m1_);                               \
        if (st_lo == (t)) poplist[rank_in(m0_)] = (uint8_t)lane;                                   \
        if (st_hi == (t) && r1_ < 64) poplist[r1_] = (uint8_t)(lane + 64);                         \
        asm volatile("" ::: "memory");                                                             \
        out = lane < (nn) ? (uint32_t)poplist[lane] : 0u;                                          \
        asm volatile("" ::: "memory");                                                             \
    }

    for (;;) {
        PA_MARK("loop_top");
        asm volatile("" : "+s"(kp) : : "memory");
        const DevIndexView ix = view_of(kp);
        const glb_u32 ec = (glb_u32)ix.ec;
        const uint32_t K = ix.k, allowed = p.allowed, spill_cap = p.spill_cap;
        if (next == end && more) {
            const uint32_t share = (ntiles > seen ? ntiles - seen : 0u) / (2 * nwaves);
            const uint32_t take = share >= 16 ? 16u : share >= 2 ? share : 2u;
            uint32_t t0 = 0;
            if (lane == 0) t0 = atomicAdd(p.tile_ctr, take);
            t0 = (uint32_t)__builtin_amdgcn_readfirstlane((int)t0) + nwaves * chunk_tiles;
            seen = t0 + take;
            if (t0 >= ntiles) more = false;
            else {
                next = (uint64_t)t0 << 6;
                end = (uint64_t)(t0 + take) << 6;
                if (end > p.n_reads) end = p.n_reads;
            }
        }
        const uint32_t st2 = (uint32_t)((lds_u16)sb)[lane];
        const uint32_t st_lo = st2 & 0xFFu, st_hi = st2 >> 8;
        const uint64_t left = end - next;
        const uint32_t nempty = PA_CNT(ST_EMPTY);
        const uint32_t nrefill = (uint32_t)(left < (uint64_t)nempty ? left : (uint64_t)nempty);
        uint32_t best = 0, sel = ST_EMPTY;
        uint32_t bestn = 0;
#define PA_CONSIDER(t, c) { const uint32_t c_ = (c); if (best < 64 && c_ > best) { best = c_; bestn = c_; sel = (t); } }
#define PA_CONSIDER_RARE_MIN(t, c, mn) { const uint32_t c_ = (c), w_ = (PA_RARE_MIN && c_ >= (mn)) ? 64u + c_ : c_; \
                                         if (best < 64 && w_ > best) { best = w_; bestn = c_; sel = (t); } }
#define PA_CONSIDER_RARE(t, c) PA_CONSIDER_RARE_MIN(t, c, PA_RARE_MIN)
        constexpr uint32_t RARE = (1u << ST_LEFT) | (1u << ST_F_LIGHT) | (1u << ST_F_SCAN) | (1u << ST_F_COOP) | (1u << ST_F_MASK);
        const bool any_rare = __ballot((((RARE >> (st_lo & 31u)) | (RARE >> (st_hi & 31u))) & 1u) != 0) != 0;
        const uint32_t n_bits_q = PA_CNT(ST_F_BITS), n_seek_q = PA_CNT(ST_SEEK), n_fwd_q = PA_CNT(ST_FWD);
        if (any_rare) {
            PA_CONSIDER_RARE_MIN(ST_F_COOP, PA_CNT(ST_F_COOP), PA_COOP_MIN)
            PA_CONSIDER_RARE(ST_F_SCAN, PA_CNT(ST_F_SCAN))
            PA_CONSIDER_RARE(ST_F_LIGHT, PA_CNT(ST_F_LIGHT))
            PA_CONSIDER_RARE(ST_F_MASK, PA_CNT(ST_F_MASK))
            PA_CONSIDER(ST_F_BITS, n_bits_q)
            PA_CONSIDER(ST_FWD, n_fwd_q)
            PA_CONSIDER_RARE(ST_LEFT, PA_CNT(ST_LEFT))
            PA_CONSIDER(ST_SEEK, n_seek_q)
            PA_CONSIDER(ST_EMPTY, nrefill)
        } else {
            const uint32_t cb = min(n_bits_q, 64u), cf = min(n_fwd_q, 64u), cs = min(n_seek_q, 64u), ce = min(nrefill, 64u);
            best = max(max(cb, cf), max(cs, ce));
            sel = cb == best ? (uint32_t)ST_F_BITS : cf == best ? (uint32_t)ST_FWD : cs == best ? (uint32_t)ST_SEEK : (uint32_t)ST_EMPTY;
            bestn = cb == best ? n_bits_q : cf == best ? n_fwd_q : cs == best ? n_seek_q : nrefill;
        }
#undef PA_CONSIDER
#undef PA_CONSIDER_RARE
#undef PA_CONSIDER_RARE_MIN
        if (best == 0) break;
#ifndef PA_SEEK_MIN
#define PA_SEEK_MIN 32u
#endif
        const bool seek_ok = n_seek_q >= PA_SEEK_MIN || n_fwd_q < 24;
        const bool dual = (sel == ST_FWD || sel == ST_SEEK) && (K <= 32 || KBIG) && n_seek_q != 0 && n_fwd_q != 0 && seek_ok && !PA_ABLATE(4u);
        if (dual) sel = ST_FWD;
        uint32_t n_own = dual ? (n_fwd_q < 64 ? n_fwd_q : 64) : bestn < 64 ? bestn : 64;
        if (PA_REFILL_ALIGN > 1 && sel == ST_EMPTY && n_own >= PA_REFILL_ALIGN && (uint64_t)n_own < left) n_own &= ~(PA_REFILL_ALIGN - 1u);
        const uint32_t n_fill = (PA_FILL && sel == ST_F_BITS && left != 0) ? (64 - n_own < nempty ? 64 - n_own : nempty) : 0u;
        const uint32_t n = n_own + n_fill;
        const uint32_t n2 = dual ? (n_seek_q < 64 ? n_seek_q : 64) : 0u;
        if (PA_DBG && lane == 0) {
            dbg[dual ? ST_DUAL : sel] += 1;
            dbg[ST_NSTAT + (dual ? ST_DUAL : sel)] += n + n2;
        }
        const unsigned long long t_sec = PA_DBG ? __builtin_readcyclecounter() : 0ull;

        PA_MARK("picked");
        const bool active = lane < n;
        uint32_t slot, slot2 = 0;
        PA_POP(sel, n_own, slot)
        if (n_fill) {
            uint32_t eslot;
            PA_POP((uint32_t)ST_EMPTY, n_fill, eslot)
            const uint32_t mine = (uint32_t)__shfl((int)eslot, (int)((lane - n_own) & 63u), 64);
            if (lane >= n_own && active) slot = mine;
        }
        const bool active2 = lane < n2;
        if (dual) PA_POP((uint32_t)ST_SEEK, n2, slot2)
        const uint32_t gslot = wave * S + slot;
        Lane s;
        {
            lane_load(s, stA, stB, stC, slot);
            s.rid = wc[2 * slot + 1];
            if (n_fill && lane >= n_own) s.lk = 0;
        }
        const ReadRef rr = GREAD ? ReadRef{p.tiles + ((uint64_t)(s.rid >> 6) * wpr) * 64 + (s.rid & 63), 64u, wpr} : ReadRef{(const uint64_t*)(rd + slot), S, wpr, true};
        const glb_u32w row = (glb_u32w)p.spill + (uint64_t)gslot * spill_cap;
        const ColRef cols{(uint32_t*)&win[slot], (uint32_t*)(wc + 2 * slot), (uint32_t*)row, (uint32_t*)(row + 4), (uint32_t*)(row + 8),
                          (uint32_t*)(row + LIST_ROW_HDR), spill_cap - LIST_ROW_HDR, (uint32_t*)row,
                          TRACE ? (uint32_t*)((glb_u32w)p.trace + (uint64_t)gslot * spill_cap) : nullptr};

        uint32_t nq2 = 0xFFu;
        PA_MARK("popped");
        const unsigned long long t_pop = PA_DBG ? __builtin_readcyclecounter() : 0ull;
        if (sel == ST_EMPTY) {
            if (active) refill_slot<GREAD>(s, next + lane, slot, kp, rd, wc, S, wpr, K);
            next += n;
        } else if (sel == ST_SEEK) {
            if (active) seek_step(s, ix, rr);
        } else if (sel == ST_FWD) {
            __builtin_amdgcn_s_waitcnt(0x0F70);
            Lane s2;
            {
#if PA_K_WIDE
                lane_load(s2, stA, stB, stC, slot2);
                if (!active2) l_zero(s2);
#else
                const u32x4 a = stA[slot2], b = stB[slot2];
                s2.lk = active2 ? a.x : 0u; s2.cm = active2 ? a.y : 0u; s2.h = active2 ? a.z : 0u; s2.of = active2 ? a.w : 0u;
                s2.rr = active2 ? b.x : 0u; s2.rm = active2 ? b.y : 0u; s2.ph = active2 ? b.z : 0u; s2.nc = active2 ? b.w : 0u;
#endif
                s2.rid = 0;
            }
            if (!active) l_zero(s);
            const uint32_t rid2 = GREAD && active2 ? wc[2 * slot2 + 1] : 0u;
            const ReadRef rr2 = GREAD ? ReadRef{p.tiles + ((uint64_t)(rid2 >> 6) * wpr) * 64 + (rid2 & 63), 64u, wpr} : ReadRef{(const uint64_t*)(rd + slot2), S, wpr};
            SeekProbe pq;
            FwdLoad fl;
            PA_MARK("dual_state2");
            pq.klo = pq.khi = pq.pending = 0; pq.v = U4{0u, 0u, NO_HANDLE, 0u};
            SeekProbe2 pq2;
            if (KBIG) {
                pq2.k0 = pq2.v0 = pq2.k1 = pq2.v1 = U4{0u, 0u, 0u, 0u}; pq2.v0.x = pq2.v1.x = NO_HANDLE; pq2.w0 = pq2.w1 = pq2.w2 = pq2.w3 = 0;
                if (n2) seek_issue_k2(s2, ix, rr2, pq2);
            }
            if (!KBIG && n2) seek_issue(s2, ix, rr2, pq);
            const bool two_l = !KBIG && active2 && seek_two(s2, K);
            const bool pairs = __popcll(__ballot(two_l)) >= 8;
            const bool two = two_l && pairs;
            SeekProbe pq1;
            pq1.klo = pq1.khi = pq1.pending = 0; pq1.v = U4{0u, 0u, NO_HANDLE, 0u};
            if (pairs) seek_issue(s2, ix, rr2, pq1, PA_SEEK_STRIDE, two);
            fwd_issue(s, ix, fl);
            __builtin_amdgcn_sched_barrier(0);
            PA_MARK("dual_issued");
            if (active2) {
                if (KBIG) seek_complete_k2(s2, K, pq2);
                else seek_complete2(s2, K, pq, two, pq1);
                nq2 = queue_of(s2, K);
                lane_store(s2, stA, stB, stC, slot2);
            }
            __builtin_amdgcn_sched_barrier(0);
            const unsigned long long t1 = PA_DBG ? __builtin_readcyclecounter() : 0ull;
            PA_MARK("dual_second");
            if (active) fwd_finish<TRACE>(s, ix, rr, cols, allowed, fl);
            PA_MARK("dual_fwd_done");
            if (PA_DBG && lane == 0) {
                const unsigned long long t3 = __builtin_readcyclecounter();
                dbg[ST_COUNT + 1] += 1; dbg[ST_COUNT + 3] += 1;
                dbg_clk[ST_COUNT + 1] += t1 - t_pop; dbg_clk[ST_COUNT + 3] += t3 - t1;
            }
            PA_MARK("dual_seek_done");
        } else if (sel == ST_LEFT) {
            if (active) left_step<TRACE>(s, ix, rr, cols, allowed);
        } else if (sel == ST_F_BITS) {
            PA_MARK("bits_begin");
            uint32_t ckey = NO_KEY;
            bool dfr = false;
            u32x4 d0{0u, 0u, 0u, 0u}, d1{0u, 0u, 0u, 0u};
            if (active && lane < n_own) {
                const bool mapped = l_st(s) != ST_NONE;
                const u32x4 w = win[slot];
                const uint32_t cand = wc[2 * slot];
                const uint32_t count = mapped ? (uint32_t)(__popc(w.y) + __popc(w.w)) : 0u;
                if (mapped && count != 0 && cand == NO_CLASS) {
                    dfr = true;
                    d0 = u32x4{s.rid, l_cov(s), l_mism(s), PA_DEFER_WINDOW | count};
                    d1 = w;
                    trace_out<TRACE>(s, true, gslot, kp);
                    s.lk = 0;
                } else {
                    const bool is_ref = mapped && count != 0;
                    if (!PA_ABLATE(1u))
                        store_result((glb_v4w)p.results + s.rid, mapped ? u32x4{l_cov(s), l_mism(s) | PA_MAPPED_BIT, is_ref ? PA_CLASS_REF | cand : 0u, count}
                                                                        : u32x4{0u, 0u, 0u, 0u});
                    trace_out<TRACE>(s, mapped, gslot, kp);
                    const glb_u32w colour_out = (glb_u32w)p.colour_out;
                    if (colour_out) colour_out[s.rid] = is_ref ? cand : NO_CLASS;
                    ckey = !mapped ? ix.num_classes + 2 : count == 0 ? ix.num_classes + 1 : cand;
                    s.lk = 0;
                }
            }
            {
                const uint64_t freed = __ballot(active && s.lk == 0);
                const uint32_t nfree = (uint32_t)__popcll(freed);
                uint32_t take = (uint32_t)(left < (uint64_t)nfree ? left : (uint64_t)nfree);
                if (PA_REFILL_ALIGN > 1 && take >= PA_REFILL_ALIGN && (uint64_t)take < left) take &= ~(PA_REFILL_ALIGN - 1u);
                if (take && !PA_ABLATE(8u)) {
                    if (active && s.lk == 0 && rank_in(freed) < take) refill_slot<GREAD>(s, next + rank_in(freed), slot, kp, rd, wc, S, wpr, K);
                    next += take;
                }
            }
            if (counting && !PA_ABLATE(2u)) append_keys(ckey, lane, kp, kchunk);
            append_deferred(dfr, d0, d1, lane, kp, dchunk);
            PA_MARK("bits_end");
        } else if (sel == ST_F_MASK) {
            const u32x4 w = active ? win[slot] : u32x4{0u, 0u, 0u, 0u};
            const uint32_t np_mine = active ? l_npend(s) : 0u;
            uint32_t a1 = w.y, a2 = w.w;
            for (uint64_t todo = __ballot(active && np_mine <= 64); todo;) {
                const uint32_t want = ((todo >> lane) & 1ull) ? np_mine : 0u;
                const uint32_t incl = wave_incl_scan(want);
                const uint32_t start = incl - want;
                const bool inpass = want != 0 && incl <= 64;
                const uint64_t pass = __ballot(inpass);
                todo &= ~pass;
                uint32_t Lr = 64, jg = 0, seg_end = 0;
                for (uint64_t m = pass; m; m &= m - 1) {
                    const uint32_t o = (uint32_t)(__ffsll((unsigned long long)m) - 1);
                    const uint32_t st = (uint32_t)__builtin_amdgcn_readlane((int)start, (int)o);
                    const uint32_t nc = (uint32_t)__builtin_amdgcn_readlane((int)np_mine, (int)o);
                    if (lane - st < nc) { Lr = o; jg = lane - st; seg_end = st + nc; }
                }
                const bool gact = Lr < 64;
                const int src = (int)(Lr & 63u);
                const uint32_t b1 = (uint32_t)__shfl((int)w.x, src, 64), b2 = (uint32_t)__shfl((int)w.z, src, 64), slotL = (uint32_t)__shfl((int)slot, src, 64);
                const glb_u32w rowL = (glb_u32w)p.spill + (uint64_t)(wave * S + slotL) * spill_cap;
                uint32_t xref = 0, xlen = 0;
                if (gact) { xref = rowL[2 * jg]; xlen = rowL[2 * jg + 1]; }
                uint32_t m1, m2;
                window_hits(ec, xref, xlen, gact, b1, b2, ix.bitmap_min, m1, m2);
                for (uint32_t o = 1; o < 64; o <<= 1) {
                    const uint32_t t1 = (uint32_t)__shfl_down((int)m1, o, 64), t2 = (uint32_t)__shfl_down((int)m2, o, 64);
                    if (gact && lane + o < seg_end) { m1 &= t1; m2 &= t2; }
                }
                const uint32_t r1 = (uint32_t)__shfl((int)m1, (int)(start & 63u), 64), r2 = (uint32_t)__shfl((int)m2, (int)(start & 63u), 64);
                if (inpass) { a1 &= r1; a2 &= r2; }
            }
            for (uint64_t todo = __ballot(active && np_mine > 64); todo; todo &= todo - 1) {
                const uint32_t Lr = (uint32_t)(__ffsll((unsigned long long)todo) - 1);
                const uint32_t b1 = (uint32_t)__shfl((int)w.x, (int)Lr, 64), b2 = (uint32_t)__shfl((int)w.z, (int)Lr, 64);
                const uint32_t npL = (uint32_t)__shfl((int)np_mine, (int)Lr, 64), slotL = (uint32_t)__shfl((int)slot, (int)Lr, 64);
                const glb_u32w rowL = (glb_u32w)p.spill + (uint64_t)(wave * S + slotL) * spill_cap;
                uint32_t r1 = 0xFFFFFFFFu, r2 = 0xFFFFFFFFu;
                for (uint32_t g = 0; g < npL; g += 64) {
                    const uint32_t ci = g + lane;
                    const bool gact = ci < npL;
                    uint32_t xref = 0, xlen = 0;
                    if (gact) { xref = rowL[2 * ci]; xlen = rowL[2 * ci + 1]; }
                    uint32_t m1, m2;
                    window_hits(ec, xref, xlen, gact, b1, b2, ix.bitmap_min, m1, m2);
                    if (gact) { r1 &= m1; r2 &= m2; }
                }
                for (uint32_t o = 32; o; o >>= 1) {
                    r1 &= (uint32_t)__shfl_xor((int)r1, (int)o, 64);
                    r2 &= (uint32_t)__shfl_xor((int)r2, (int)o, 64);
                }
                if (lane == Lr) { a1 &= r1; a2 &= r2; }
            }
            if (active) {
                if (a1 != w.y || a2 != w.w) wc[2 * slot] = NO_CLASS;
                win[slot] = u32x4{w.x, a1, w.z, a2};
                s.nc = (s.nc & ~NC_COL_MASK) | 1u;
                l_set_st(s, ST_F_BITS);
            }
        } else if (sel == ST_F_SCAN) {
            Isect is;
            is.base_len = is.base_ref = is.base_colour = 0;
            if (active) isect_pick(s, cols, is);
            const uint32_t ncol_mine = l_ncol(s);
            if (active && ncol_mine > 3) is.base_colour = ec[4ull * is.base_ref];
            uint32_t my_alive = 0;
            for (uint64_t todo = __ballot(active && ncol_mine > 0 && ncol_mine <= 64); todo;) {
                const uint32_t want = ((todo >> lane) & 1ull) ? ncol_mine : 0u;
                const uint32_t incl = wave_incl_scan(want);
                const uint32_t start = incl - want;
                const bool inpass = want != 0 && incl <= 64;
                const uint64_t pass = __ballot(inpass);
                todo &= ~pass;
                uint32_t Lr = 64, jg = 0;
                for (uint64_t m = pass; m; m &= m - 1) {
                    const uint32_t o = (uint32_t)(__ffsll((unsigned long long)m) - 1);
                    const uint32_t st = (uint32_t)__builtin_amdgcn_readlane((int)start, (int)o);
                    const uint32_t nc = (uint32_t)__builtin_amdgcn_readlane((int)ncol_mine, (int)o);
                    if (lane - st < nc) { Lr = o; jg = lane - st; }
                }
                const bool gact = Lr < 64;
                const int src = (int)(Lr & 63u);
                const uint32_t bref = (uint32_t)__shfl((int)is.base_ref, src, 64), blen = (uint32_t)__shfl((int)is.base_len, src, 64),
                               slotL = (uint32_t)__shfl((int)slot, src, 64);
                const glb_u32w rowL = (glb_u32w)p.spill + (uint64_t)(wave * S + slotL) * spill_cap;
                const glb_v4 brec = (glb_v4)(ec + 4ull * bref);
                const u32x4 q0 = brec[0], q1 = brec[1], q2 = brec[2];
                const uint32_t b[8] = {q0.y, q0.z, q0.w, q1.x, q1.y, q1.z, q1.w, blen > 7 ? q2.x : 0xFFFFFFFFu};
                uint32_t xref = bref, xlen = 0;
                if (gact) {
                    if (jg < LDS_CLASSES) { xref = rowL[jg]; xlen = rowL[4 + jg]; }
                    else { const u32x4 qd = *(glb_v4)(rowL + LIST_ROW_HDR + 4 * (jg - LDS_CLASSES)); xref = qd.x; xlen = qd.y; }
                }
                const bool mine = xref != bref;
// ... 222 lines not shown
```

Before: 13.51 billion reads/s.

## Add compact quotient-filter pair dictionary for k<=24 k-mer lookups

Introduces a new hash dictionary layout for k<=24 indices: two 64-bit entries per bucket, holding a quotient-style remainder tag, handle and offset, built by inserting with an atomic min on displacement ordering. The seek path gets pair-specific issue/complete routines and a PAIR kernel template variant, which is selected when the index was built with pairs. The aim is to shrink the table and cut the memory traffic per lookup compared with the multi-slot buckets. It limits handles to 24 bits and offsets to 11 bits, and it adds a displacement-based probing loop plus rebuild retries when displacement overflows.

```diff
diff --git a/__graft_entry__.py b/__graft_entry__.py
--- a/__graft_entry__.py
+++ b/__graft_entry__.py
@@ -14,6 +14,7 @@
     _b = importlib.import_module("rust-pseudoaligner_amd._build")
     _b.build_product()
     _b.build_maxbins_variant()
+    _b.build_pairknobs_variant()
     _b.build_abi_check()
     import helpers
     helpers.build_all()
diff --git a/rust-pseudoaligner_amd/_build.py b/rust-pseudoaligner_amd/_build.py
--- a/rust-pseudoaligner_amd/_build.py
+++ b/rust-pseudoaligner_amd/_build.py
@@ -82,6 +82,22 @@
     return MAXBINS_SO
 
 
+PAIRKNOBS_SO = OBJ_DIR / "libpseudoaligner_amd_pairknobs.so"
+
+
+def build_pairknobs_variant(force: bool = False) -> Path:
+    build_product()
+    hipcc = hipcc_path()
+    src = CSRC / "device_flatten.cpp"
+    obj = OBJ_DIR / "device_flatten.pairknobs.o"
+    if force or _stale(obj, _deps_of(src)):
+        _run([hipcc, "--offload-arch=gfx950", "-O3", "-std=c++17", "-fPIC", "-pthread", "-Wall", "-Wno-unused-function", "-DPA_DEBUG_KNOBS", "-x", "hip", "-c", str(src), "-o", str(obj)])
+    objs = [OBJ_DIR / (s + ".o") for s in HOST_SOURCES + HIP_SOURCES if s != "device_flatten.cpp"] + [obj]
+    if force or _stale(PAIRKNOBS_SO, objs):
+        _run([hipcc, "--offload-arch=gfx950", "-shared", "-fPIC", "-pthread"] + [str(o) for o in objs] + ["-ldl", "-lz", "-o", str(PAIRKNOBS_SO)])
+    return PAIRKNOBS_SO
+
+
 ABI_CHECK_SRC = ROOT / "integration" / "c" / "abi_check.c"
 ABI_CHECK_BIN = ROOT / "integration" / "c" / "abi_check"
 
diff --git a/rust-pseudoaligner_amd/csrc/device_flatten.cpp b/rust-pseudoaligner_amd/csrc/device_flatten.cpp
--- a/rust-pseudoaligner_amd/csrc/device_flatten.cpp
+++ b/rust-pseudoaligner_amd/csrc/device_flatten.cpp
@@ -18,6 +18,7 @@
     DevIndexView v;
     v.table = table.data();
     v.nbuckets = nbuckets;
+    v.dict_pairs = dict_pairs;
     v.blobs = blobs.data();
     v.ledge = ledge.data();
     v.seg_g = seg_g.data();
@@ -39,6 +40,24 @@
     return v;
 }
 
+uint32_t dict_pair_log2(uint32_t k, uint64_t nblocks, uint64_t nk, uint32_t bump) {
+    uint64_t max_blocks = PAIR_MAX_BLOCKS;
+    double load = PAIR_LOAD;
+    uint32_t b = PAIR_MIN_LOG2;
+    if (const char* v = knob_str("PA_PAIR_MAX_BLOCKS")) max_blocks = std::min<uint64_t>(max_blocks, strtoull(v, nullptr, 10));
+    if (const char* v = knob_str("PA_PAIR_LOAD")) { const double x = atof(v); if (x > 0.01 && x <= 1.9) load = x; }
+    if (k > PAIR_MAX_K || nblocks >= max_blocks) return 0;
+    if (knob_str("PA_DICT_LOAD")) return 0;
+    while (b < PAIR_MAX_LOG2 && (double)nk > load * (double)(1ull << b)) ++b;
+    if (const char* v = knob_str("PA_PAIR_LOG2")) {
+        const uint32_t x = (uint32_t)atoi(v);
+        if (x == 0) return 0;
+        b = std::min(std::max(x, PAIR_MIN_LOG2), PAIR_MAX_LOG2);
+    }
+    b += bump;
+    return b <= PAIR_MAX_LOG2 ? b : 0;
+}
+
 namespace {
 
 template <class F>
@@ -97,22 +116,25 @@
     }
 };
 
-struct HostAtomics {
-    static bool cas(uint32_t* p, uint32_t expect, uint32_t v) { return __atomic_compare_exchange_n(p, &expect, v, false, __ATOMIC_RELAXED, __ATOMIC_RELAXED); }
-    static void and_(uint32_t* p, uint32_t m) { __atomic_fetch_and(p, m, __ATOMIC_RELAXED); }
-};
-
 template <>
 struct Dict<uint64_t> {
     static constexpr double LOAD = DICT_LOAD;
     static constexpr uint32_t SLOTS = SLOTS_PER_BUCKET;
     uint32_t* words;
     uint64_t nbuckets;
-    void insert_mt(uint64_t kmer, uint32_t handle, uint32_t off) { dict_insert_home<HostAtomics>(words, (uint32_t)nbuckets, kmer, handle, off); }
-    void insert_rest_mt(uint64_t kmer, uint32_t handle, uint32_t off) { dict_insert_rest<HostAtomics>(words, (uint32_t)nbuckets, kmer, handle, off); }
+    uint32_t pairs = 0;
+    std::atomic<uint32_t>* far = nullptr;
+    void insert_mt(uint64_t kmer, uint32_t handle, uint32_t off) {
+        if (!pairs) dict_insert_home<HostAtomics>(words, (uint32_t)nbuckets, kmer, handle, off);
+        else if (!pair_insert<HostAtomics>(reinterpret_cast<uint64_t*>(words), pairs, kmer, handle, off)) far->store(1);
+    }
+    void insert_rest_mt(uint64_t kmer, uint32_t handle, uint32_t off) {
+        if (!pairs) dict_insert_rest<HostAtomics>(words, (uint32_t)nbuckets, kmer, handle, off);
+        else pair_flag<HostAtomics>(reinterpret_cast<uint64_t*>(words), pairs, kmer);
+    }
     bool find(uint64_t kmer, uint32_t& handle, uint32_t& off, uint32_t* probes_out = nullptr) const {
         uint32_t probes = 0;
-        const bool found = dict_find64(words, (uint32_t)nbuckets, kmer, handle, off, probes);
+        const bool found = dict_find64(words, (uint32_t)nbuckets, pairs, kmer, handle, off, probes);
         if (probes_out) *probes_out = probes;
         return found;
     }
@@ -527,24 +549,31 @@
     }
     double load0 = Dict<KT>::LOAD;
     if (const char* v = knob_str("PA_DICT_LOAD")) { const double x = atof(v); if (x > 0.01 && x <= 0.95) load0 = x; }
-    for (double load = load0; !device_dict; load *= 0.75) {
-        out.nbuckets = std::max<uint64_t>(1, (uint64_t)((double)nk / (Dict<KT>::SLOTS * load)) + 1);
+    uint32_t bump = 0;
+    std::atomic<uint32_t> pair_far{0};
+    bool try_pairs = sizeof(KT) == 8;
+    for (double load = load0; !device_dict; out.dict_pairs ? (void)++bump : (void)(load *= 0.75)) {
+        out.dict_pairs = try_pairs ? dict_pair_log2(k, nblocks, nk, bump) : 0;
+        if (!out.dict_pairs) try_pairs = false;
+        out.nbuckets = out.dict_pairs ? 1ull << out.dict_pairs : std::max<uint64_t>(1, (uint64_t)((double)nk / (Dict<KT>::SLOTS * load)) + 1);
         if (out.nbuckets >= 0xFFFFFFFFull) return fail(PA_ERR_UNSUPPORTED, "dictionary exceeds 2^32 buckets");
-        out.table.assign(out.nbuckets * BUCKET_WORDS, 0xFFFFFFFFu);
+        out.table.assign(dict_table_words(out.nbuckets, out.dict_pairs), 0xFFFFFFFFu);
         dict = Dict<KT>{out.table.data(), out.nbuckets};
+        if constexpr (sizeof(KT) == 8) { dict.pairs = out.dict_pairs; dict.far = &pair_far; pair_far.store(0); }
         par_ranges(threads, N, [&](uint64_t a, uint64_t b, int) {
             for (uint64_t i = a; i < b; ++i) node_kmers((uint32_t)i, [&](KT km, uint32_t h, uint32_t o) { dict.insert_mt(km, h, o); });
         });
         par_ranges(threads, N, [&](uint64_t a, uint64_t b, int) {
             for (uint64_t i = a; i < b; ++i) node_kmers((uint32_t)i, [&](KT km, uint32_t h, uint32_t o) { dict.insert_rest_mt(km, h, o); });
         });
+        if (pair_far.load()) continue;
         std::atomic<uint32_t> bad{NO_HANDLE}, far{0};
         par_ranges(threads, N, [&](uint64_t a, uint64_t b, int) {
             for (uint64_t i = a; i < b; ++i)
                 node_kmers((uint32_t)i, [&](KT km, uint32_t h, uint32_t o) {
                     uint32_t fh, fo, probes = 0;
                     if (!dict.find(km, fh, fo, &probes) || fh != h || fo != o) bad.store((uint32_t)i);
-                    if (probes > DICT_MAX_PROBES) far.store(1);
+                    if (!out.dict_pairs && probes > DICT_MAX_PROBES) far.store(1);
                 });
         });
         if (bad.load() != NO_HANDLE) return fail(PA_ERR_FORMAT, "a k-mer of node %u occurs twice in the graph", bad.load());
diff --git a/rust-pseudoaligner_amd/csrc/device_flatten.hpp b/rust-pseudoaligner_amd/csrc/device_flatten.hpp
--- a/rust-pseudoaligner_amd/csrc/device_flatten.hpp
+++ b/rust-pseudoaligner_amd/csrc/device_flatten.hpp
@@ -11,6 +11,7 @@
 struct FlatDevice {
     std::vector<uint32_t> table;
     uint64_t nbuckets = 0;
+    uint32_t dict_pairs = 0;
     std::vector<uint8_t> blobs;
     std::vector<uint32_t> handle;
     std::vector<uint32_t> node_s;
@@ -32,8 +33,10 @@
 
 int flatten_for_device(const pa_flat_index& f, int threads, FlatDevice& out, bool device_dict = false);
 
+uint32_t dict_pair_log2(uint32_t k, uint64_t nblocks, uint64_t nk, uint32_t bump);
+
 #ifdef __HIPCC__
-int device_fill_index(const FlatDevice& fd, const uint8_t* d_blobs, DeviceBuffer<uint32_t>& table, uint64_t* nbuckets);
+int device_fill_index(const FlatDevice& fd, const uint8_t* d_blobs, DeviceBuffer<uint32_t>& table, uint64_t* nbuckets, uint32_t* dict_pairs);
 #endif
 
 }
diff --git a/rust-pseudoaligner_amd/csrc/device_index.hip b/rust-pseudoaligner_amd/csrc/device_index.hip
--- a/rust-pseudoaligner_amd/csrc/device_index.hip
+++ b/rust-pseudoaligner_amd/csrc/device_index.hip
@@ -176,7 +176,7 @@
     if (idx->num_cus <= 0) idx->num_cus = 256;
     rc = upload(idx->d_blobs, fd.blobs);
     if (rc == PA_OK) rc = upload(idx->d_ledge, fd.ledge);
-    if (rc == PA_OK) rc = device_fill_index(fd, idx->d_blobs.get(), idx->d_table, &fd.nbuckets);
+    if (rc == PA_OK) rc = device_fill_index(fd, idx->d_blobs.get(), idx->d_table, &fd.nbuckets, &fd.dict_pairs);
     if (rc == PA_OK) rc = upload(idx->d_seg_g, fd.seg_g);
     if (rc == PA_OK) rc = upload(idx->d_seg_nid, fd.seg_nid);
     if (rc == PA_OK) rc = upload(idx->d_ec, fd.ec);
@@ -199,11 +199,11 @@
     idx->dv.class_ref = idx->d_class_ref.get();
     idx->dv.class_len = idx->d_class_len.get();
     idx->dv.wtable = idx->d_wtable.get();
-    idx->dv.stream_nt = (fd.k <= 32 && fd.nbuckets * BUCKET_WORDS * 4 > (512ull << 20)) ? 1u : 0u;
+    idx->dv.stream_nt = (fd.k <= 32 && dict_table_words(fd.nbuckets, fd.dict_pairs) * 4 > (512ull << 20)) ? 1u : 0u;
     pa_index_stats& s = idx->stats;
     s.num_kmers = fd.num_kmers;
-    s.table_slots = fd.nbuckets * SLOTS_PER_BUCKET;
-    s.bytes_table = fd.nbuckets * BUCKET_WORDS * 4;
+    s.table_slots = dict_table_words(fd.nbuckets, fd.dict_pairs) / SLOT_WORDS;
+    s.bytes_table = dict_table_words(fd.nbuckets, fd.dict_pairs) * 4;
     s.bytes_graph = fd.blobs.size() + fd.ledge.size() * 4 + fd.seg_g.size() * 12;
     s.bytes_classes = (fd.ec.size() + fd.class_ref.size() + fd.class_len.size() + ctab.size() + fd.wtable.size()) * 4;
     s.bytes_total = s.bytes_table + s.bytes_graph + s.bytes_classes;
@@ -232,6 +232,44 @@
         }
     }
     return PA_OK;
+}
+
+int padbg_dict_table(const pa_flat_index* flat, int device, uint32_t builds, void* out, uint64_t cap, uint64_t* bytes, uint32_t* dict_pairs, uint32_t* differing) {
+    if (!flat || !bytes || !dict_pairs || !differing) return fail(PA_ERR_INVALID_ARG, "null argument");
+    FlatDevice fd;
+    int threads = usable_threads();
+    if (threads < 1) threads = 1;
+    *differing = 0;
+    if (device < 0) {
+        const int rc = flatten_for_device(*flat, threads, fd, false);
+        if (rc != PA_OK) return rc;
+        *bytes = fd.table.size() * 4;
+        *dict_pairs = fd.dict_pairs;
+        if (out && cap >= *bytes) memcpy(out, fd.table.data(), *bytes);
+        return PA_OK;
+    }
+    int rc = use_device(device);
+    if (rc == PA_OK) rc = flatten_for_device(*flat, threads, fd, true);
+    DeviceBuffer<uint8_t> d_blobs;
+    if (rc == PA_OK) rc = upload(d_blobs, fd.blobs);
+    std::vector<uint8_t> again;
+    for (uint32_t i = 0; rc == PA_OK && i < builds; ++i) {
+        DeviceBuffer<uint32_t> d_table;
+        rc = device_fill_index(fd, d_blobs.get(), d_table, &fd.nbuckets, &fd.dict_pairs);
+        if (rc != PA_OK) break;
+        const uint64_t n = dict_table_words(fd.nbuckets, fd.dict_pairs) * 4;
+        if (i == 0) {
+            *bytes = n;
+            *dict_pairs = fd.dict_pairs;
+            if (!out || cap < n) return PA_OK;
+            if (hipMemcpy(out, d_table.get(), n, hipMemcpyDeviceToHost) != hipSuccess) return fail(PA_ERR_HIP, "hipMemcpy failed");
+        } else {
+            again.resize(n);
+            if (hipMemcpy(again.data(), d_table.get(), n, hipMemcpyDeviceToHost) != hipSuccess) return fail(PA_ERR_HIP, "hipMemcpy failed");
+            if (n != *bytes || memcmp(again.data(), out, n) != 0) ++*differing;
+        }
+    }
+    return rc;
 }
 
 int pa_index_get_stats(const pa_index* idx, pa_index_stats* stats) {
diff --git a/rust-pseudoaligner_amd/csrc/device_layout.hpp b/rust-pseudoaligner_amd/csrc/device_layout.hpp
--- a/rust-pseudoaligner_amd/csrc/device_layout.hpp
+++ b/rust-pseudoaligner_amd/csrc/device_layout.hpp
@@ -45,6 +45,46 @@
 constexpr uint32_t SLOT_FLAG_OVERFLOW = 8u;
 constexpr double DICT_LOAD = 0.25;
 constexpr uint32_t DICT_MAX_PROBES = 15;
+constexpr uint32_t PAIR_KEY_BITS = 48, PAIR_MAX_K = 24;
+constexpr uint32_t PAIR_MIN_LOG2 = 21;
+constexpr uint32_t PAIR_MAX_LOG2 = 31;
+#ifndef PA_PAIR_LOAD
+#define PA_PAIR_LOAD 0.5
+#endif
+constexpr double PAIR_LOAD = PA_PAIR_LOAD;
+constexpr uint32_t PAIR_HANDLE_BITS = 24, PAIR_NO_HANDLE = 0xFFFFFFu, PAIR_OFF_SHIFT = 24, PAIR_OFF_MASK = 0x7FFu;
+constexpr uint32_t PAIR_FLAG_BIT = 35, PAIR_TAG_SHIFT = 36, PAIR_TAG_BITS = 28;
+constexpr uint32_t PAIR_MAX_BLOCKS = PAIR_NO_HANDLE;
+constexpr uint64_t PAIR_EMPTY = ~0ull, PAIR_KEY_MASK = (1ull << PAIR_KEY_BITS) - 1;
+constexpr uint64_t PAIR_MUL1 = 0x9E3779B1ull, PAIR_MUL2 = 0x85EBCA77ull;
+constexpr uint64_t pair_mul_inverse(uint64_t a) {
+    uint64_t x = a;
+    for (int i = 0; i < 6; ++i) x *= 2 - a * x;
+    return x & PAIR_KEY_MASK;
+}
+constexpr uint64_t PAIR_INV1 = pair_mul_inverse(PAIR_MUL1), PAIR_INV2 = pair_mul_inverse(PAIR_MUL2);
+PA_HD uint64_t pair_mix(uint64_t x) {
+    x ^= x >> 24;
+    x = (x * PAIR_MUL1) & PAIR_KEY_MASK;
+    x ^= x >> 24;
+    return (x * PAIR_MUL2) & PAIR_KEY_MASK;
+}
+PA_HD uint64_t pair_unmix(uint64_t m) {
+    m = (m * PAIR_INV2) & PAIR_KEY_MASK;
+    m ^= m >> 24;
+    m = (m * PAIR_INV1) & PAIR_KEY_MASK;
+    return m ^ (m >> 24);
+}
+constexpr uint32_t PAIR_MAX_DISP = 254;
+PA_HD uint32_t pair_max_disp(uint32_t b) { return b >= 28 ? PAIR_MAX_DISP : (1u << (b - 20)) - 2u; }
+PA_HD uint64_t pair_entry(uint32_t tag, uint32_t handle, uint32_t off) {
+    return ((uint64_t)tag << PAIR_TAG_SHIFT) | (1ull << PAIR_FLAG_BIT) | ((uint64_t)off << PAIR_OFF_SHIFT) | handle;
+}
+PA_HD uint32_t pair_entry_tag(uint64_t e) { return (uint32_t)(e >> PAIR_TAG_SHIFT); }
+PA_HD uint32_t pair_entry_handle(uint64_t e) { return (uint32_t)e & PAIR_NO_HANDLE; }
+PA_HD uint32_t pair_entry_off(uint64_t e) { return (uint32_t)(e >> PAIR_OFF_SHIFT) & PAIR_OFF_MASK; }
+
+PA_HD uint64_t dict_table_words(uint64_t nbuckets, uint32_t dict_pairs) { return nbuckets * (dict_pairs ? 4u : BUCKET_WORDS); }
 
 struct alignas(16) U4 {
     uint32_t x, y, z, w;
@@ -75,6 +115,7 @@
     uint32_t stream_nt;
     uint32_t bitmap_min;
     uint32_t bitmap_words;
+    uint32_t dict_pairs;
 };
 
 PA_HD uint32_t class_record_chunks(uint32_t len) { return len < 4 ? 2u : (len + 4) >> 2; }
diff --git a/rust-pseudoaligner_amd/csrc/dict_slots.hpp b/rust-pseudoaligner_amd/csrc/dict_slots.hpp
--- a/rust-pseudoaligner_amd/csrc/dict_slots.hpp
+++ b/rust-pseudoaligner_amd/csrc/dict_slots.hpp
@@ -2,6 +2,17 @@
 #include "lane_steps.hpp"
 
 namespace pa {
+
+struct HostAtomics {
+    static bool cas(uint32_t* p, uint32_t expect, uint32_t v) { return __atomic_compare_exchange_n(p, &expect, v, false, __ATOMIC_RELAXED, __ATOMIC_RELAXED); }
+    static void and_(uint32_t* p, uint32_t m) { __atomic_fetch_and(p, m, __ATOMIC_RELAXED); }
+    static uint64_t min64(uint64_t* p, uint64_t v) {
+        uint64_t old = __atomic_load_n(p, __ATOMIC_RELAXED);
+        while (old > v && !__atomic_compare_exchange_n(p, &old, v, false, __ATOMIC_RELAXED, __ATOMIC_RELAXED)) {}
+        return old;
+    }
+    static void and64(uint64_t* p, uint64_t m) { __atomic_fetch_and(p, m, __ATOMIC_RELAXED); }
+};
 
 template <class A>
 PA_HD bool slot_claim(uint32_t* slot, uint64_t km, uint32_t handle, uint32_t off) {
@@ -60,4 +71,68 @@
     return false;
 }
 
+
+template <class A>
+PA_HD bool pair_insert(uint64_t* table, uint32_t b, uint64_t km, uint32_t handle, uint32_t off) {
+    const uint32_t rbits = PAIR_KEY_BITS - b, mask = (uint32_t)((1ull << b) - 1), maxd = pair_max_disp(b);
+    const uint64_t m = pair_mix(km);
+    uint32_t p = (uint32_t)(m >> rbits);
+    uint64_t w = pair_entry((uint32_t)m & ((1u << rbits) - 1u), handle, off);
+    for (;;) {
+        uint64_t* e = table + 2ull * p;
+        uint64_t old = A::min64(e, w);
+        if (old > w) w = old;
+        if (w == PAIR_EMPTY) return true;
+        old = A::min64(e + 1, w);
+        if (old > w) w = old;
+        if (w == PAIR_EMPTY) return true;
+        if ((pair_entry_tag(w) >> rbits) >= maxd) return false;
+        w += 1ull << (PAIR_TAG_SHIFT + rbits);
+        p = (p + 1) & mask;
+    }
 }
+
+PA_HD uint32_t pair_locate(const uint64_t* table, uint32_t b, uint64_t km, uint64_t& entry) {
+    const uint32_t rbits = PAIR_KEY_BITS - b, mask = (uint32_t)((1ull << b) - 1), maxd = pair_max_disp(b);
+    const uint64_t m = pair_mix(km);
+    const uint32_t q = (uint32_t)(m >> rbits), r = (uint32_t)m & ((1u << rbits) - 1u);
+    for (uint32_t d = 0; d <= maxd; ++d) {
+        const uint64_t* e = table + 2ull * ((q + d) & mask);
+        const uint32_t want = r | (d << rbits);
+        for (uint32_t i = 0; i < 2; ++i) {
+            const uint64_t w = e[i];
+            if (pair_entry_tag(w) == want) { entry = w; return d; }
+        }
+    }
+    return NO_HANDLE;
+}
+
+template <class A>
+PA_HD void pair_flag(uint64_t* table, uint32_t b, uint64_t km) {
+    uint64_t w;
+    const uint32_t d = pair_locate(table, b, km, w);
+    if (d == NO_HANDLE || d == 0) return;
+    const uint32_t mask = (uint32_t)((1ull << b) - 1), q = (uint32_t)(pair_mix(km) >> (PAIR_KEY_BITS - b));
+    for (uint32_t j = 0; j < d; ++j) A::and64(table + 2ull * ((q + j) & mask), ~(1ull << PAIR_FLAG_BIT));
+}
+
+PA_HD bool pair_find64(const uint64_t* table, uint32_t b, uint64_t km, uint32_t& handle, uint32_t& off, uint32_t& probes) {
+    const uint32_t rbits = PAIR_KEY_BITS - b, mask = (uint32_t)((1ull << b) - 1), maxd = pair_max_disp(b);
+    const uint64_t m = pair_mix(km);
+    const uint32_t q = (uint32_t)(m >> rbits), r = (uint32_t)m & ((1u << rbits) - 1u);
+    for (probes = 0;; ++probes) {
+        const uint64_t* e = table + 2ull * ((q + probes) & mask);
+        const uint64_t e0 = e[0], e1 = e[1];
+        const uint32_t want = r | (probes << rbits);
+        if (pair_entry_tag(e0) == want) { handle = pair_entry_handle(e0); off = pair_entry_off(e0); return true; }
+        if (pair_entry_tag(e1) == want) { handle = pair_entry_handle(e1); off = pair_entry_off(e1); return true; }
+        if (((e0 >> PAIR_FLAG_BIT) & 1u) || probes >= maxd) return false;
+    }
+}
+
+PA_HD bool dict_find64(const uint32_t* table, uint32_t nbuckets, uint32_t dict_pairs, uint64_t km, uint32_t& handle, uint32_t& off, uint32_t& probes) {
+    if (dict_pairs) return pair_find64(reinterpret_cast<const uint64_t*>(table), dict_pairs, km, handle, off, probes);
+    return dict_find64(table, nbuckets, km, handle, off, probes);
+}
+
+}
diff --git a/rust-pseudoaligner_amd/csrc/index_fill.hip b/rust-pseudoaligner_amd/csrc/index_fill.hip
--- a/rust-pseudoaligner_amd/csrc/index_fill.hip
+++ b/rust-pseudoaligner_amd/csrc/index_fill.hip
@@ -27,6 +27,8 @@
 struct DeviceAtomics {
     __device__ static bool cas(uint32_t* p, uint32_t expect, uint32_t v) { return atomicCAS(p, expect, v) == expect; }
     __device__ static void and_(uint32_t* p, uint32_t m) { atomicAnd(p, m); }
+    __device__ static uint64_t min64(uint64_t* p, uint64_t v) { return atomicMin(reinterpret_cast<unsigned long long*>(p), (unsigned long long)v); }
+    __device__ static void and64(uint64_t* p, uint64_t m) { atomicAnd(reinterpret_cast<unsigned long long*>(p), (unsigned long long)m); }
 };
 template <> struct FillOps<u128> {
     static constexpr uint32_t SLOTS = 2;
@@ -62,13 +64,13 @@
 };
 
 template <class KT>
-__device__ __forceinline__ bool dict_find(const uint32_t* table, uint32_t nbuckets, KT km, uint32_t& handle, uint32_t& off, uint32_t& probes);
+__device__ __forceinline__ bool dict_find(const uint32_t* table, uint32_t nbuckets, uint32_t pairs, KT km, uint32_t& handle, uint32_t& off, uint32_t& probes);
 template <>
-__device__ __forceinline__ bool dict_find<uint64_t>(const uint32_t* table, uint32_t nbuckets, uint64_t km, uint32_t& handle, uint32_t& off, uint32_t& probes) {
-    return dict_find64(table, nbuckets, km, handle, off, probes);
+__device__ __forceinline__ bool dict_find<uint64_t>(const uint32_t* table, uint32_t nbuckets, uint32_t pairs, uint64_t km, uint32_t& handle, uint32_t& off, uint32_t& probes) {
+    return dict_find64(table, nbuckets, pairs, km, handle, off, probes);
 }
 template <>
-__device__ __forceinline__ bool dict_find<u128>(const uint32_t* table, uint32_t nbuckets, u128 km, uint32_t& handle, uint32_t& off, uint32_t& probes) {
+__device__ __forceinline__ bool dict_find<u128>(const uint32_t* table, uint32_t nbuckets, uint32_t, u128 km, uint32_t& handle, uint32_t& off, uint32_t& probes) {
     uint32_t b = FillOps<u128>::bucket(km, nbuckets);
     for (probes = 0; probes < nbuckets; ++probes) {
         const int r = FillOps<u128>::look(table + (uint64_t)b * BUCKET_WORDS, km, handle, off);
@@ -107,13 +109,16 @@
 template <class KT>
 __global__ __launch_bounds__(256) void pa_fill_insert_kernel(const uint8_t* __restrict__ blobs, const uint32_t* __restrict__ handle, const uint32_t* __restrict__ node_s,
                                                              const uint64_t* __restrict__ kcum, uint32_t num_nodes, uint64_t nk, uint32_t k, uint32_t* table,
-                                                             uint32_t nbuckets, int pass) {
+                                                             uint32_t nbuckets, int pass, uint32_t pairs, uint32_t* __restrict__ flags) {
     const uint64_t g = (uint64_t)blockIdx.x * blockDim.x + threadIdx.x;
     if (g >= nk) return;
     const KmerAt a = kmer_at(blobs, handle, node_s, kcum, num_nodes, g, k);
     const KT km = FillOps<KT>::get(a.seq, a.rel, k);
     if constexpr (sizeof(KT) == 8) {
-        if (pass == 0) dict_insert_home<DeviceAtomics>(table, nbuckets, km, a.block, a.off);
+        if (pairs) {
+            if (pass != 0) pair_flag<DeviceAtomics>(reinterpret_cast<uint64_t*>(table), pairs, km);
+            else if (!pair_insert<DeviceAtomics>(reinterpret_cast<uint64_t*>(table), pairs, km, a.block, a.off)) flags[1] = 1;
+        } else if (pass == 0) dict_insert_home<DeviceAtomics>(table, nbuckets, km, a.block, a.off);
         else dict_insert_rest<DeviceAtomics>(table, nbuckets, km, a.block, a.off);
     } else {
         if (pass != 0) return;
@@ -128,18 +133,19 @@
 template <class KT>
 __global__ __launch_bounds__(256) void pa_fill_verify_kernel(const uint8_t* __restrict__ blobs, const uint32_t* __restrict__ handle, const uint32_t* __restrict__ node_s,
                                                              const uint64_t* __restrict__ kcum, uint32_t num_nodes, uint64_t nk, uint32_t k,
-                                                             const uint32_t* __restrict__ table, uint32_t nbuckets, uint32_t* __restrict__ flags) {
+                                                             const uint32_t* __restrict__ table, uint32_t nbuckets, uint32_t pairs, uint32_t* __restrict__ flags) {
     const uint64_t g = (uint64_t)blockIdx.x * blockDim.x + threadIdx.x;
     if (g >= nk) return;
     const KmerAt a = kmer_at(blobs, handle, node_s, kcum, num_nodes, g, k);
     const KT km = FillOps<KT>::get(a.seq, a.rel, k);
     uint32_t fh = 0, fo = 0, probes = 0;
-    if (!dict_find<KT>(table, nbuckets, km, fh, fo, probes) || fh != a.block || fo != a.off) atomicMin(flags, a.node);
-    if (probes > DICT_MAX_PROBES) flags[1] = 1;
-}
-
-template <class KT>
-int fill_t(const FlatDevice& fd, const uint8_t* d_blobs, DeviceBuffer<uint32_t>& table_out, uint64_t* nbuckets_out) {
+    if (pairs && flags[1]) return;
+    if (!dict_find<KT>(table, nbuckets, pairs, km, fh, fo, probes) || fh != a.block || fo != a.off) atomicMin(flags, a.node);
+    if (!pairs && probes > DICT_MAX_PROBES) flags[1] = 1;
+}
+
+template <class KT>
+int fill_t(const FlatDevice& fd, const uint8_t* d_blobs, DeviceBuffer<uint32_t>& table_out, uint64_t* nbuckets_out, uint32_t* pairs_out) {
     const uint32_t N = fd.num_nodes, k = fd.k;
     const uint64_t nk = fd.num_kmers;
     DeviceBuffer<uint32_t> table, d_handle, d_node_s, d_flags;
@@ -154,28 +160,35 @@
     PA_HIP_TRY(hipMemcpy(d_kcum.get(), fd.node_kcum.data(), ((size_t)N + 1) * 8, hipMemcpyHostToDevice));
     uint64_t nbuckets = 0;
     double load0 = FillOps<KT>::LOAD;
+    size_t free_b = 0, total_b = 0;
+    const bool mem_known = hipMemGetInfo(&free_b, &total_b) == hipSuccess;
     {
-        size_t free_b = 0, total_b = 0;
         const double dense = sizeof(KT) == 8 ? 0.5 : FillOps<KT>::LOAD;
-        if (load0 < dense && hipMemGetInfo(&free_b, &total_b) == hipSuccess && (double)nk / (FillOps<KT>::SLOTS * load0) * BUCKET_WORDS * 4 > (double)free_b / 4) load0 = dense;
+        if (load0 < dense && mem_known && (double)nk / (FillOps<KT>::SLOTS * load0) * BUCKET_WORDS * 4 > (double)free_b / 4) load0 = dense;
     }
     if (const char* v = knob_str("PA_DICT_LOAD")) { const double x = atof(v); if (x > 0.01 && x <= 0.95) load0 = x; }
-    for (double load = load0;; load *= 0.75) {
-        nbuckets = std::max<uint64_t>(1, (uint64_t)((double)nk / (FillOps<KT>::SLOTS * load)) + 1);
+    uint32_t pairs = 0, bump = 0;
+    const uint64_t nblocks = fd.blobs.size() / CH_BLOCK;
+    bool try_pairs = sizeof(KT) == 8;
+    for (double load = load0;; pairs ? (void)++bump : (void)(load *= 0.75)) {
+        pairs = try_pairs ? dict_pair_log2(k, nblocks, nk, bump) : 0;
+        if (pairs && mem_known && (double)(16ull << pairs) > (double)free_b / 4) pairs = 0;
+        if (!pairs) try_pairs = false;
+        nbuckets = pairs ? 1ull << pairs : std::max<uint64_t>(1, (uint64_t)((double)nk / (FillOps<KT>::SLOTS * load)) + 1);
         if (nbuckets >= 0xFFFFFFFFull) return fail(PA_ERR_UNSUPPORTED, "dictionary exceeds 2^32 buckets");
-        if ((e = table.alloc(nbuckets * BUCKET_WORDS)) != PA_OK) return e;
-        PA_HIP_TRY(hipMemsetAsync(table.get(), 0xFF, nbuckets * BUCKET_WORDS * 4, nullptr));
+        if ((e = table.alloc(dict_table_words(nbuckets, pairs))) != PA_OK) return e;
+        PA_HIP_TRY(hipMemsetAsync(table.get(), 0xFF, dict_table_words(nbuckets, pairs) * 4, nullptr));
         const uint32_t init[4] = {NO_HANDLE, 0u, NO_HANDLE, NO_HANDLE};
         PA_HIP_TRY(hipMemcpy(d_flags.get(), init, 16, hipMemcpyHostToDevice));
         if (nk) {
             const dim3 grid((uint32_t)((nk + 255) / 256));
             for (int pass = 0; pass < (sizeof(KT) == 8 ? 2 : 1); ++pass) {
                 hipLaunchKernelGGL(pa_fill_insert_kernel<KT>, grid, dim3(256), 0, nullptr, d_blobs, d_handle.get(), d_node_s.get(), d_kcum.get(), N, nk, k,
-                                   table.get(), (uint32_t)nbuckets, pass);
+                                   table.get(), (uint32_t)nbuckets, pass, pairs, d_flags.get());
                 PA_HIP_TRY(hipGetLastError());
             }
             hipLaunchKernelGGL(pa_fill_verify_kernel<KT>, grid, dim3(256), 0, nullptr, d_blobs, d_handle.get(), d_node_s.get(), d_kcum.get(), N, nk, k,
-                               table.get(), (uint32_t)nbuckets, d_flags.get());
+                               table.get(), (uint32_t)nbuckets, pairs, d_flags.get());
             PA_HIP_TRY(hipGetLastError());
         }
         uint32_t flags[4];
@@ -184,14 +197,15 @@
         if (!flags[1]) break;
     }
     *nbuckets_out = nbuckets;
+    *pairs_out = pairs;
     table_out = std::move(table);
     return PA_OK;
 }
 
 }
 
-int device_fill_index(const FlatDevice& fd, const uint8_t* d_blobs, DeviceBuffer<uint32_t>& table, uint64_t* nbuckets) {
-    return fd.k <= 32 ? fill_t<uint64_t>(fd, d_blobs, table, nbuckets) : fill_t<u128>(fd, d_blobs, table, nbuckets);
-}
-
-}
+int device_fill_index(const FlatDevice& fd, const uint8_t* d_blobs, DeviceBuffer<uint32_t>& table, uint64_t* nbuckets, uint32_t* dict_pairs) {
+    return fd.k <= 32 ? fill_t<uint64_t>(fd, d_blobs, table, nbuckets, dict_pairs) : fill_t<u128>(fd, d_blobs, table, nbuckets, dict_pairs);
+}
+
+}
diff --git a/rust-pseudoaligner_amd/csrc/lane_steps_body.hpp b/rust-pseudoaligner_amd/csrc/lane_steps_body.hpp
--- a/rust-pseudoaligner_amd/csrc/lane_steps_body.hpp
+++ b/rust-pseudoaligner_amd/csrc/lane_steps_body.hpp
@@ -540,6 +540,44 @@
     if (seek_settle(s, K, q0, two)) return;
     (void)seek_settle(s, K, q1, false);
 }
+PA_HD uint32_t l_disp(const Lane& s) { return l_probe(s) | (l_pending(s) << 4); }
+PA_HD bool seek_two_pair(const Lane& s, uint32_t K) { return (l_flags(s) & F_SPEC) && l_disp(s) == 0 && l_kp(s) + PA_SEEK_STRIDE <= l_L(s) - K; }
+PA_HD void seek_issue_pair(const Lane& s, const DevIndexView& ix, ReadRef rd, SeekProbe& q, uint32_t ahead = 0, bool live = true) {
+    const uint32_t at = live ? l_kp(s) + ahead : l_kp(s);
+    const uint64_t m = pair_mix(read_window_in(rd, at) & ix.kmask);
+    const uint32_t b = ix.dict_pairs, rbits = PAIR_KEY_BITS - b, d = ahead ? 0u : l_disp(s);
+    uint32_t pr = ((uint32_t)(m >> rbits) + d) & ((1u << b) - 1u);
+    if (!live) pr = 0;
+    q.v = ld_stream(reinterpret_cast<const U4*>(ix.table) + pr, (PA_NT & 4) || ix.stream_nt);
+    q.klo = (((uint32_t)m & ((1u << rbits) - 1u)) | (d << rbits)) << (PAIR_TAG_SHIFT - 32);
+    q.khi = d < pair_max_disp(b) ? 1u << (PAIR_FLAG_BIT - 32) : 0u;
+    q.pending = 0;
+}
+PA_HD bool seek_settle_pair(Lane& s, uint32_t K, const SeekProbe& q, bool more) {
+    const uint32_t low = (1u << (PAIR_TAG_SHIFT - 32)) - 1u;
+    const bool h0 = (q.v.y ^ q.klo) <= low, h1 = (q.v.w ^ q.klo) <= low;
+    const uint32_t lo = h0 ? q.v.x : q.v.z, hi = h0 ? q.v.y : q.v.w;
+    const uint32_t h = (h0 || h1) ? lo & PAIR_NO_HANDLE : NO_HANDLE, off = ((lo >> PAIR_OFF_SHIFT) | (hi << (32 - PAIR_OFF_SHIFT))) & PAIR_OFF_MASK;
+    const bool full = (~q.v.y & q.khi) != 0;
+    if (h == NO_HANDLE && full) {
+        const uint32_t d = l_disp(s) + 1u;
+        s.nc = (s.nc & ~(15u << NC_PROBE_SHIFT)) | ((d & 15u) << NC_PROBE_SHIFT);
+        s.rm = (s.rm & ~SK_MASK) | (d >> 4);
+        return true;
+    }
+    if (!more || h != NO_HANDLE) {
+        seek_finish(s, K, h, off, false, 0u);
+        return true;
+    }
+    l_set_kp(s, l_kp(s) + PA_SEEK_STRIDE);
+    s.rm &= ~SK_MASK;
+    s.nc &= ~(15u << NC_PROBE_SHIFT);
+    return false;
+}
+PA_HD void seek_complete2_pair(Lane& s, uint32_t K, const SeekProbe& q0, bool two, const SeekProbe& q1) {
+    if (seek_settle_pair(s, K, q0, two)) return;
+    (void)seek_settle_pair(s, K, q1, false);
+}
 PA_HD void seek_finish(Lane& s, uint32_t K, uint32_t h, uint32_t off, bool full, uint32_t probe) {
     const uint32_t L = l_L(s), kp = l_kp(s);
     s.nc &= ~(15u << NC_PROBE_SHIFT);
@@ -595,7 +633,7 @@
                h1 = q.k1.x == q.w0 && q.k1.y == q.w1 && q.k1.z == q.w2 && q.k1.w == q.w3 && q.v1.x != NO_HANDLE;
     seek_finish(s, K, h0 ? q.v0.x : h1 ? q.v1.x : NO_HANDLE, h0 ? q.v0.y : q.v1.y, q.v0.x != NO_HANDLE && q.v1.x != NO_HANDLE, l_probe(s));
 }
-PA_HD void seek_step(Lane& s, const DevIndexView& ix, ReadRef rd) {
+PA_HD void seek_step_slots(Lane& s, const DevIndexView& ix, ReadRef rd) {
     const uint32_t K = ix.k;
     if (K > 32) {
         SeekProbe2 q2;
@@ -608,6 +646,17 @@
     seek_issue(s, ix, rd, q);
     seek_issue(s, ix, rd, q1, PA_SEEK_STRIDE, two);
     seek_complete2(s, K, q, two, q1);
+}
+PA_HD void seek_step_pair(Lane& s, const DevIndexView& ix, ReadRef rd) {
+    SeekProbe q, q1;
+    const bool two = seek_two_pair(s, ix.k);
+    seek_issue_pair(s, ix, rd, q);
+    seek_issue_pair(s, ix, rd, q1, PA_SEEK_STRIDE, two);
+    seek_complete2_pair(s, ix.k, q, two, q1);
+}
+PA_HD void seek_step(Lane& s, const DevIndexView& ix, ReadRef rd) {
+    if (ix.dict_pairs) seek_step_pair(s, ix, rd);
+    else seek_step_slots(s, ix, rd);
 }
 #endif
 
diff --git a/rust-pseudoaligner_amd/csrc/map_pool.hip b/rust-pseudoaligner_amd/csrc/map_pool.hip
--- a/rust-pseudoaligner_amd/csrc/map_pool.hip
+++ b/rust-pseudoaligner_amd/csrc/map_pool.hip
@@ -49,7 +49,7 @@
     DevIndexView v;
     v.table = p->ix.table; v.nbuckets = p->ix.nbuckets; v.blobs = p->ix.blobs; v.ledge = p->ix.ledge;
     v.seg_g = p->ix.seg_g; v.seg_nid = p->ix.seg_nid; v.ec = p->ix.ec; v.class_ref = p->ix.class_ref; v.class_len = p->ix.class_len;
-    v.wtable = p->ix.wtable; v.wbuckets = p->ix.wbuckets; v.kmask = p->ix.kmask; v.kmask_hi = p->ix.kmask_hi; v.k = p->ix.k; v.num_nodes = p->ix.num_nodes; v.num_classes = p->ix.num_classes; v.num_segs = p->ix.num_segs; v.stream_nt = p->ix.stream_nt; v.bitmap_min = p->ix.bitmap_min; v.bitmap_words = p->ix.bitmap_words;
+    v.wtable = p->ix.wtable; v.wbuckets = p->ix.wbuckets; v.kmask = p->ix.kmask; v.kmask_hi = p->ix.kmask_hi; v.k = p->ix.k; v.num_nodes = p->ix.num_nodes; v.num_classes = p->ix.num_classes; v.num_segs = p->ix.num_segs; v.stream_nt = p->ix.stream_nt; v.bitmap_min = p->ix.bitmap_min; v.bitmap_words = p->ix.bitmap_words; v.dict_pairs = p->ix.dict_pairs;
     return v;
 }
 
@@ -255,15 +255,22 @@
 
 int launch_map_pool(const MapParams& p, uint32_t grid, size_t lds_bytes, hipStream_t stream) {
     const bool gread = p.wpr > PA_LDS_READ_WORDS;
+    const bool pair = p.ix.dict_pairs != 0;
+    if (gread && pair) return p.trace ? launch_kernel(&wide::pa_map_pool_kernel<true, true, false, false, false, true>, p, grid, lds_bytes, stream)
+                                      : launch_kernel(&wide::pa_map_pool_kernel<false, true, false, false, false, true>, p, grid, lds_bytes, stream);
     if (gread) return p.trace ? launch_kernel(&wide::pa_map_pool_kernel<true, true, false, false>, p, grid, lds_bytes, stream)
                               : launch_kernel(&wide::pa_map_pool_kernel<false, true, false, false>, p, grid, lds_bytes, stream);
-    if (p.trace) return launch_kernel(&narrow::pa_map_pool_kernel<true, false, false, false>, p, grid, lds_bytes, stream);
+    if (p.trace) return pair ? launch_kernel(&narrow::pa_map_pool_kernel<true, false, false, false, false, true>, p, grid, lds_bytes, stream)
+                             : launch_kernel(&narrow::pa_map_pool_kernel<true, false, false, false>, p, grid, lds_bytes, stream);
 #ifdef PA_DEBUG_KNOBS
-    if (p.dbg || p.ablate) return launch_kernel(&narrow::pa_map_pool_kernel<false, false, true, false>, p, grid, lds_bytes, stream);
+    if (p.dbg || p.ablate) return pair ? launch_kernel(&narrow::pa_map_pool_kernel<false, false, true, false, false, true>, p, grid, lds_bytes, stream)
+                                       : launch_kernel(&narrow::pa_map_pool_kernel<false, false, true, false>, p, grid, lds_bytes, stream);
 #endif
     if (p.ix.k > 32)
         return p.pool_slots == 128 ? launch_kernel(&narrow::pa_map_pool_kernel<false, false, false, true, true>, p, grid, lds_bytes, stream)
                                    : launch_kernel(&narrow::pa_map_pool_kernel<false, false, false, false, true>, p, grid, lds_bytes, stream);
+    if (pair) return p.pool_slots == 128 ? launch_kernel(&narrow::pa_map_pool_kernel<false, false, false, true, false, true>, p, grid, lds_bytes, stream)
+                                         : launch_kernel(&narrow::pa_map_pool_kernel<false, false, false, false, false, true>, p, grid, lds_bytes, stream);
     if (p.pool_slots == 128) return launch_kernel(&narrow::pa_map_pool_kernel<false, false, false, true>, p, grid, lds_bytes, stream);
     return launch_kernel(&narrow::pa_map_pool_kernel<false, false, false, false>, p, grid, lds_bytes, stream);
 }
diff --git a/rust-pseudoaligner_amd/csrc/map_pool_kernel.inc b/rust-pseudoaligner_amd/csrc/map_pool_kernel.inc
--- a/rust-pseudoaligner_amd/csrc/map_pool_kernel.inc
+++ b/rust-pseudoaligner_amd/csrc/map_pool_kernel.inc
@@ -107,7 +107,7 @@
 #ifndef PA_MAP_MIN_BLOCKS
 #define PA_MAP_MIN_BLOCKS 3
 #endif
-template <bool TRACE, bool GREAD, bool DBG, bool S128 = false, bool KBIG = false>
+template <bool TRACE, bool GREAD, bool DBG, bool S128 = false, bool KBIG = false, bool PAIR = false>
 __global__ __launch_bounds__(PA_MAP_BLOCK, PA_MAP_MIN_BLOCKS) void pa_map_pool_kernel(const MapParams p_arg) {
     karg_ptr kp = (karg_ptr)__builtin_amdgcn_kernarg_segment_ptr();
     (void)p_arg;
@@ -269,7 +269,10 @@
             if (active) refill_slot<GREAD>(s, next + lane, slot, kp, rd, wc, S, wpr, K);
             next += n;
         } else if (sel == ST_SEEK) {
-            if (active) seek_step(s, ix, rr);
+            if (active) {
+                if (PAIR) seek_step_pair(s, ix, rr);
+                else seek_step_slots(s, ix, rr);
+            }
         } else if (sel == ST_FWD) {
             __builtin_amdgcn_s_waitcnt(0x0F70);
             Lane s2;
@@ -296,18 +299,21 @@
                 pq2.k0 = pq2.v0 = pq2.k1 = pq2.v1 = U4{0u, 0u, 0u, 0u}; pq2.v0.x = pq2.v1.x = NO_HANDLE; pq2.w0 = pq2.w1 = pq2.w2 = pq2.w3 = 0;
                 if (n2) seek_issue_k2(s2, ix, rr2, pq2);
             }
-            if (!KBIG && n2) seek_issue(s2, ix, rr2, pq);
-            const bool two_l = !KBIG && active2 && seek_two(s2, K);
+            if (PAIR && n2) seek_issue_pair(s2, ix, rr2, pq);
+            if (!KBIG && !PAIR && n2) seek_issue(s2, ix, rr2, pq);
+            const bool two_l = !KBIG && active2 && (PAIR ? seek_two_pair(s2, K) : seek_two(s2, K));
             const bool pairs = __popcll(__ballot(two_l)) >= 8;
             const bool two = two_l && pairs;
             SeekProbe pq1;
             pq1.klo = pq1.khi = pq1.pending = 0; pq1.v = U4{0u, 0u, NO_HANDLE, 0u};
-            if (pairs) seek_issue(s2, ix, rr2, pq1, PA_SEEK_STRIDE, two);
+            if (PAIR && pairs) seek_issue_pair(s2, ix, rr2, pq1, PA_SEEK_STRIDE, two);
+            if (!PAIR && pairs) seek_issue(s2, ix, rr2, pq1, PA_SEEK_STRIDE, two);
             fwd_issue(s, ix, fl);
             __builtin_amdgcn_sched_barrier(0);
             PA_MARK("dual_issued");
             if (active2) {
                 if (KBIG) seek_complete_k2(s2, K, pq2);
+                else if (PAIR) seek_complete2_pair(s2, K, pq, two, pq1);
                 else seek_complete2(s2, K, pq, two, pq1);
                 nq2 = queue_of(s2, K);
                 lane_store(s2, stA, stB, stC, slot2);
```

Result: faster. 13.97 billion reads/s, median of 6 (+3.4%).
